# SymbioticLab/Oobleck

Measured on AMD Instinct MI355X. Metric: tokens/sec (whole node) GPT-2 1F1B, higher is better.
Workload: dtype bf16; 1 GPU; gpt2.yaml GPT-2-small 1F1B, global microbatch 128x1024 tokens, bf16; model=gpt2, global_batch=128, seq_len=1024, parallelism=pp1dp1

## Files before the change

### include/oobleck_stage.h

```cpp
#ifndef OOBLECK_STAGE_H
#define OOBLECK_STAGE_H

#include <stdint.h>

#ifdef __cplusplus
extern "C" {
#endif

enum {
  OB_KIND_EMBED = 0,
  OB_KIND_BLOCK = 1,
  OB_KIND_FINAL = 2
};

typedef struct ob_layer* ob_layer_t;

typedef struct {
  int32_t kind;
  int32_t n_embd;
  int32_t n_head;
  int32_t n_positions;
  int32_t vocab_size;
  int32_t max_batch;
  int32_t seq_len;
  int32_t n_slots;
  int32_t dtype;
} ob_layer_desc;

int64_t ob_layer_param_count(const ob_layer_desc* desc);

int ob_layer_create(const ob_layer_desc* desc, ob_layer_t* out);

enum {
  OB_DROP_EMBD = 0,
  OB_DROP_ATTN = 1,
  OB_DROP_RESID_ATTN = 2,
  OB_DROP_RESID_MLP = 3
};

typedef struct {
  float embd_pdrop;
  float resid_pdrop;
  float attn_pdrop;
  int32_t layer_id;
  uint64_t seed;
} ob_dropout_desc;

int ob_layer_create_ex(const ob_layer_desc* desc, const ob_dropout_desc* drop,
                       ob_layer_t* out);

int ob_layer_uses_flash(ob_layer_t l);
int ob_flash_eligible(const ob_layer_desc* desc, float attn_pdrop);

int ob_layer_plan_query(const ob_layer_desc* desc,
                        const ob_dropout_desc* drop, int modes, int64_t* out,
                        int cap);

int ob_layer_set_training(ob_layer_t l, int on);

int ob_layer_set_dropout_tick(ob_layer_t l, uint64_t tick);

int ob_layer_bind(ob_layer_t l, void* params, void* grads);

int ob_layer_set_batch(ob_layer_t l, int32_t batch);

int ob_layer_forward(ob_layer_t l, int32_t slot, const void* in, void* out,
                     const int64_t* labels, void* stream);

int ob_layer_backward(ob_layer_t l, int32_t slot, const void* dout, void* din,
                      void* stream);

int ob_layer_destroy(ob_layer_t l);

int ob_layer_refresh_weights(ob_layer_t l, void* stream);

int ob_adamw_step(void* p, const void* g, void* m, void* v, int64_t n,
                  int32_t step, float lr, float beta1, float beta2, float eps,
                  float weight_decay, void* stream);


int64_t ob_sqnorm_ws_count(const int64_t* counts, int32_t n);

int ob_sqnorm_multi_f32(const void* const* ptrs, const int64_t* counts,
                        const int32_t* out_index, int32_t n, void* ws,
                        void* out, void* stream);

int ob_clip_finish(const void* sq, int32_t n, float max_norm, void* stats,
                   void* stream);

int ob_adamw_step_scaled(void* p, const void* g, void* m, void* v, int64_t n,
                         int32_t step, float lr, float beta1, float beta2,
                         float eps, float weight_decay, const void* clip_stats,
                         void* stream);


int ob_gemm_f32(int transA, int transB, int64_t M, int64_t N, int64_t K,
                float alpha, const void* A, int64_t lda,
                int64_t strideA1, int64_t strideA2,
                const void* B, int64_t ldb,
                int64_t strideB1, int64_t strideB2,
                float beta, void* C, int64_t ldc,
                int64_t strideC1, int64_t strideC2,
                int64_t n1, int64_t n2,
                const void* bias, const void* residual, int atomic, int splitk,
                void* stream);

int ob_layernorm_fwd_f32(const void* x, const void* w, const void* b, void* y,
                         void* mean, void* rstd, int64_t rows, int64_t H,
                         float eps, void* stream);
int ob_layernorm_bwd_f32(const void* x, const void* w, const void* mean,
                         const void* rstd, const void* dy, void* dx,
                         void* dw, void* db, int64_t rows, int64_t H,
                         int dx_accum, void* stream);

int ob_softmax_causal_fwd_f32(void* scores, int64_t batch, int64_t S,
                              float scale, void* stream);
int ob_softmax_causal_bwd_f32(const void* P, void* dP, int64_t batch,
                              int64_t S, void* stream);

int ob_gelu_fwd_f32(const void* u, void* g, int64_t n, void* stream);
int ob_gelu_bwd_f32(const void* u, const void* dg, void* du, int64_t n,
                    void* stream);

int ob_colsum_f32(const void* X, void* db, int64_t M, int64_t N, void* stream);

int ob_dropout_mask(uint64_t seed, int32_t layer_id, int32_t site,
                    uint64_t tick, float p, int64_t n, void* keep_u8,
                    void* stream);
int ob_dropout_scale_f32(uint64_t seed, int32_t layer_id, int32_t site,
                         uint64_t tick, float p, const void* x, void* y,
                         int64_t n, void* stream);
int ob_dropout_scale_bf16(uint64_t seed, int32_t layer_id, int32_t site,
                          uint64_t tick, float p, const void* x, void* y,
                          int64_t n, void* stream);
int ob_dropout_add_f32(uint64_t seed, int32_t layer_id, int32_t site,
                       uint64_t tick, float p, const void* t, const void* res,
                       void* y, int64_t n, void* stream);
int ob_dropout_add_bf16(uint64_t seed, int32_t layer_id, int32_t site,
                        uint64_t tick, float p, const void* t,
                        const void* res, void* y, int64_t n, void* stream);
int ob_dropout_scale_colsum_f32(uint64_t seed, int32_t layer_id, int32_t site,
                                uint64_t tick, float p, const void* dy,
                                void* dm, void* db, int64_t M, int64_t N,
                                void* stream);
int ob_dropout_scale_colsum_bf16(uint64_t seed, int32_t layer_id, int32_t site,
                                 uint64_t tick, float p, const void* dy,
                                 void* dm, void* db, int64_t M, int64_t N,
                                 void* stream);

int ob_gemm_bf16(int transA, int transB, int64_t M, int64_t N, int64_t K,
                 float alpha, const void* A, int64_t lda,
                 int64_t strideA1, int64_t strideA2,
                 const void* B, int64_t ldb,
                 int64_t strideB1, int64_t strideB2,
                 float beta, void* C, int64_t ldc,
                 int64_t strideC1, int64_t strideC2,
                 int64_t n1, int64_t n2,
                 const void* bias, const void* residual, int out_kind,
                 int splitk, void* stream);
int ob_gemm_bf16_route(int transA, int transB, int64_t M, int64_t N, int64_t K,
                       int64_t n1, int64_t n2, int out_kind, int splitk,
                       float beta, int aligned16, int env_mask,
                       const char* force, int32_t* out);

int ob_layer_lt_shapes(const ob_layer_desc* desc, int64_t* out, int cap);
int ob_gemm_lt_tune(const int64_t* shape);
int ob_gemm_lt_choice(const int64_t* shape, double* out, char* top1_name,
                      char* chosen_name, int name_cap);
int ob_gemm_lt_candidates(const int64_t* shape, int32_t* index, int32_t* pos,
                          double* us, int cap);
int64_t ob_gemm_lt_table_size(void);
int64_t ob_gemm_lt_untuned_uses(void);
int ob_gemm_lt_plan_index(const int64_t* shape, void* stream);

int ob_flash_fwd_nt_bf16(const void* qkv, void* O, void* lse, int64_t B,
                         int64_t Sq, int64_t H, int64_t nh, float scale,
                         void* stream);
int ob_flash_bwd_nt_bf16(const void* qkv, const void* dO, const void* lse,
                         const void* D, void* dqkv, void* dbias_qkv,
                         int64_t B, int64_t Sq, int64_t H, int64_t nh,
                         float scale, void* stream);
int ob_flash_bwd_nt_d_bf16(const void* qkv, const void* O, const void* dO,
                           const void* lse, void* D_ws, void* dqkv,
                           void* dbias_qkv, int64_t B, int64_t Sq, int64_t H,
                           int64_t nh, float scale, void* stream);
int ob_flash_fwd_nt_drop_bf16(const void* qkv, void* O, void* lse, int64_t B,
                              int64_t Sq, int64_t H, int64_t nh, float scale,
                              uint64_t seed, int32_t layer_id, uint64_t tick,
                              float p, void* stream);
int ob_flash_bwd_nt_d_drop_bf16(const void* qkv, const void* O, const void* dO,
                                const void* lse, void* D_ws, void* dqkv,
                                void* dbias_qkv, int64_t B, int64_t Sq,
                                int64_t H, int64_t nh, float scale,
                                uint64_t seed, int32_t layer_id, uint64_t tick,
                                float p, void* stream);
int ob_flash_fold_rows(int64_t kind, int64_t Sq, int64_t block, int64_t unit,
                       int64_t* row0, int64_t* first_tile, int64_t* n_tiles);
int64_t ob_flash_fold_grid(int64_t kind, int64_t Sq, int64_t Z);
int ob_flash_fold_id(int64_t kind, int64_t Sq, int64_t Z, int64_t id,
                     int64_t* z, int64_t* block);

int ob_set_deterministic(int on);
int ob_deterministic(void);

enum {
  OB_DET_WS_COLSUM = 0,
  OB_DET_WS_GELU = 1,
  OB_DET_WS_LN = 2,
  OB_DET_WS_DROP_CS = 3,
  OB_DET_WS_CE = 4
};
int64_t ob_det_ws_count(int which, int64_t M, int64_t N);
int ob_colsum_det_bf16(const void* X, void* db, int64_t M, int64_t N,
                       void* ws, void* stream);
int ob_gelu_bwd_colsum_det_bf16(const void* u, const void* dg, void* du,
                                void* db, int64_t M, int64_t N, void* ws,
                                void* stream);
int ob_layernorm_bwd_res_det_bf16(const void* x, const void* w,
                                  const void* mean, const void* rstd,
                                  const void* dy, const void* res, void* dx,
                                  void* dw, void* db, void* sum_res,
                                  void* sum_dx, int64_t rows, int64_t H,
                                  void* ws, void* stream);
int ob_dropout_scale_colsum_det_bf16(uint64_t seed, int32_t layer_id,
                                     int32_t site, uint64_t tick, float p,
                                     const void* dy, void* dm, void* db,
                                     int64_t M, int64_t N, void* ws,
                                     void* stream);
int ob_ce_fwd_det_bf16(const void* logits, const void* labels, void* lse,
                       void* loss, int64_t B, int64_t Sq, int64_t V,
                       int64_t ld, void* ws, void* stream);
int ob_embed_bwd_det_bf16(const void* ids, const void* dout, void* dwte,
                          void* dwpe, int64_t B, int64_t Sq, int64_t H,
                          void* stream);
int ob_embed_bwd_drop_det_bf16(uint64_t seed, int32_t layer_id, int32_t site,
                               uint64_t tick, float p, const void* ids,
                               const void* dout, void* dwte, void* dwpe,
                               int64_t B, int64_t Sq, int64_t H, void* stream);
int ob_colpart_finish_f32(const void* part, int64_t nblk, int64_t N,
                          int64_t ld, void* dst, void* stream);

int ob_f32_to_bf16(const void* x, void* y, int64_t n, void* stream);
int ob_f32_to_bf16_t(const void* x, void* y, int64_t rows, int64_t cols,
                     void* stream);
int ob_bf16_to_f32(const void* x, void* y, int64_t n, void* stream);

void ob_profile_enable(int on);
void ob_profile_reset(void);
int ob_profile_read(int fam, double* total_ms, long long* count);

const char* ob_last_error(void);

const char* ob_build_arch(void);

#ifdef __cplusplus
}
#endif
#endif
```

### oobleck_amd/_ext.py

```python
from __future__ import annotations

import ctypes
import pathlib

_LIB = None
SO_PATH = pathlib.Path(__file__).resolve().parent / "libob_stage.so"


class ObLayerDesc(ctypes.Structure):
    _fields_ = [
        ("kind", ctypes.c_int32),
        ("n_embd", ctypes.c_int32),
        ("n_head", ctypes.c_int32),
        ("n_positions", ctypes.c_int32),
        ("vocab_size", ctypes.c_int32),
        ("max_batch", ctypes.c_int32),
        ("seq_len", ctypes.c_int32),
        ("n_slots", ctypes.c_int32),
        ("dtype", ctypes.c_int32),
    ]


class ObDropoutDesc(ctypes.Structure):
    _fields_ = [
        ("embd_pdrop", ctypes.c_float),
        ("resid_pdrop", ctypes.c_float),
        ("attn_pdrop", ctypes.c_float),
        ("layer_id", ctypes.c_int32),
        ("seed", ctypes.c_uint64),
    ]


DROP_EMBD, DROP_ATTN, DROP_RESID_ATTN, DROP_RESID_MLP = 0, 1, 2, 3


def _configure(lib: ctypes.CDLL) -> ctypes.CDLL:
    i64, i32, f32, vp = ctypes.c_int64, ctypes.c_int32, ctypes.c_float, ctypes.c_void_p
    lib.ob_last_error.restype = ctypes.c_char_p
    lib.ob_build_arch.restype = ctypes.c_char_p
    lib.ob_layer_param_count.restype = i64
    lib.ob_layer_param_count.argtypes = [ctypes.POINTER(ObLayerDesc)]
    lib.ob_layer_create.argtypes = [ctypes.POINTER(ObLayerDesc),
                                    ctypes.POINTER(vp)]
    u64 = ctypes.c_uint64
    lib.ob_layer_create_ex.argtypes = [ctypes.POINTER(ObLayerDesc),
                                       ctypes.POINTER(ObDropoutDesc),
                                       ctypes.POINTER(vp)]
    lib.ob_layer_set_training.argtypes = [vp, i32]
    lib.ob_layer_uses_flash.argtypes = [vp]
    lib.ob_flash_eligible.argtypes = [ctypes.POINTER(ObLayerDesc), f32]
    lib.ob_layer_plan_query.argtypes = [ctypes.POINTER(ObLayerDesc),
                                        ctypes.POINTER(ObDropoutDesc), i32,
                                        ctypes.POINTER(i64), i32]
    lib.ob_layer_set_dropout_tick.argtypes = [vp, u64]
    key = [u64, i32, i32, u64, f32]
    lib.ob_dropout_mask.argtypes = key + [i64, vp, vp]
    lib.ob_dropout_scale_f32.argtypes = key + [vp, vp, i64, vp]
    lib.ob_dropout_scale_bf16.argtypes = key + [vp, vp, i64, vp]
    lib.ob_dropout_add_f32.argtypes = key + [vp, vp, vp, i64, vp]
    lib.ob_dropout_add_bf16.argtypes = key + [vp, vp, vp, i64, vp]
    lib.ob_dropout_scale_colsum_f32.argtypes = key + [vp, vp, vp, i64, i64, vp]
    lib.ob_dropout_scale_colsum_bf16.argtypes = key + [vp, vp, vp, i64, i64,
                                                       vp]
    lib.ob_layer_bind.argtypes = [vp, vp, vp]
    lib.ob_layer_set_batch.argtypes = [vp, i32]
    lib.ob_layer_forward.argtypes = [vp, i32, vp, vp, vp, vp]
    lib.ob_layer_backward.argtypes = [vp, i32, vp, vp, vp]
    lib.ob_layer_destroy.argtypes = [vp]
    lib.ob_layer_refresh_weights.argtypes = [vp, vp]
    lib.ob_adamw_step.argtypes = [vp, vp, vp, vp, i64, i32, f32, f32, f32,
                                  f32, f32, vp]
    lib.ob_sqnorm_ws_count.restype = i64
    lib.ob_sqnorm_ws_count.argtypes = [ctypes.POINTER(i64), i32]
    lib.ob_sqnorm_multi_f32.argtypes = [ctypes.POINTER(vp),
                                        ctypes.POINTER(i64),
                                        ctypes.POINTER(i32), i32, vp, vp, vp]
    lib.ob_clip_finish.argtypes = [vp, i32, f32, vp, vp]
    lib.ob_adamw_step_scaled.argtypes = [vp, vp, vp, vp, i64, i32, f32, f32,
                                         f32, f32, f32, vp, vp]
    lib.ob_gemm_f32.argtypes = [i32, i32, i64, i64, i64, f32, vp, i64, i64,
                                i64, vp, i64, i64, i64, f32, vp, i64, i64,
                                i64, i64, i64, vp, vp, i32, i32, vp]
    lib.ob_layernorm_fwd_f32.argtypes = [vp, vp, vp, vp, vp, vp, i64, i64,
                                         f32, vp]
    lib.ob_layernorm_bwd_f32.argtypes = [vp, vp, vp, vp, vp, vp, vp, vp, i64,
                                         i64, i32, vp]
    lib.ob_softmax_causal_fwd_f32.argtypes = [vp, i64, i64, f32, vp]
    lib.ob_softmax_causal_bwd_f32.argtypes = [vp, vp, i64, i64, vp]
    lib.ob_gelu_fwd_f32.argtypes = [vp, vp, i64, vp]
    lib.ob_gelu_bwd_f32.argtypes = [vp, vp, vp, i64, vp]
    lib.ob_colsum_f32.argtypes = [vp, vp, i64, i64, vp]
    lib.ob_gemm_bf16.argtypes = [i32, i32, i64, i64, i64, f32, vp, i64, i64,
                                 i64, vp, i64, i64, i64, f32, vp, i64, i64,
                                 i64, i64, i64, vp, vp, i32, i32, vp]
    lib.ob_f32_to_bf16.argtypes = [vp, vp, i64, vp]
    lib.ob_f32_to_bf16_t.argtypes = [vp, vp, i64, i64, vp]
    lib.ob_f32_to_bf16_t_ld.argtypes = [vp, vp, i64, i64, i64, vp]
    lib.ob_bf16_to_f32.argtypes = [vp, vp, i64, vp]
    lib.ob_gelu_fwd_bf16.argtypes = [vp, vp, i64, vp]
    lib.ob_gelu_bwd_bf16.argtypes = [vp, vp, vp, i64, vp]
    lib.ob_ce_fwd_bf16.argtypes = [vp, vp, vp, vp, i64, i64, i64, i64, vp]
    lib.ob_ce_bwd_bf16.argtypes = [vp, vp, vp, vp, i64, i64, i64, i64, vp]
    lib.ob_embed_fwd_bf16.argtypes = [vp, vp, vp, vp, i64, i64, i64, vp]
    lib.ob_embed_bwd_bf16.argtypes = [vp, vp, vp, vp, i64, i64, i64, vp]
    lib.ob_softmax_causal_fwd_bf16.argtypes = [vp, i64, i64, f32, vp]
    lib.ob_softmax_causal_bwd_bf16.argtypes = [vp, vp, i64, i64, vp]
    lib.ob_transpose_bf16.argtypes = [vp, vp, i64, i64, vp]
    lib.ob_gemm_lt_bias.argtypes = [i32, i32, i64, i64, i64, f32, vp, i64,
                                    vp, i64, f32, vp, i64, i32, vp, vp]
    lib.ob_gemm_lt_f32.argtypes = [i32, i32, i64, i64, i64, f32, vp, i64,
                                   vp, i64, f32, vp, i64, vp]
    lib.ob_flash_fwd_bf16.argtypes = [vp, vp, vp, vp, i64, i64, i64, i64,
                                      f32, vp]
    lib.ob_transpose_bf16_b.argtypes = [vp, vp, i64, i64, i64, i64, i64,
                                        i64, i64, vp]
    lib.ob_layernorm_fwd_bf16.argtypes = [vp, vp, vp, vp, vp, vp, i64, i64,
                                          f32, vp]
    lib.ob_layernorm_bwd_bf16.argtypes = [vp, vp, vp, vp, vp, vp, vp, vp,
                                          i64, i64, i32, vp]
    lib.ob_colsum_bf16.argtypes = [vp, vp, i64, i64, vp]
    lib.ob_layernorm_fwd_copy_bf16.argtypes = [vp, vp, vp, vp, vp, vp, vp,
                                               i64, i64, f32, vp]
    lib.ob_layernorm_bwd_res_bf16.argtypes = [vp, vp, vp, vp, vp, vp, vp, vp,
                                              vp, vp, vp, i64, i64, vp]
    lib.ob_gelu_bwd_colsum_bf16.argtypes = [vp, vp, vp, vp, i64, i64, vp]
    lib.ob_gemm_lt.argtypes = [i32, i32, i64, i64, i64, f32, vp, i64, vp,
                               i64, f32, vp, i64, i32, vp]
    lib.ob_gemm_bf16_nt_8ph.argtypes = [vp, vp, vp, vp, vp, i64, i64, i64,
                                        i64, i64, i64, i64, i64, i64, i64,
                                        i64, i64, i64, i64, f32, f32, i32,
                                        i32, vp, i64]
    lib.ob_gemm_bf16_route.argtypes = [i32, i32, i64, i64, i64, i64, i64, i32,
                                       i32, f32, i32, i32, ctypes.c_char_p,
                                       ctypes.POINTER(ctypes.c_int32)]
    lib.ob_gemm_lt_bias_res.argtypes = [i32, i32, i64, i64, i64, f32, vp, i64,
                                        vp, i64, vp, i64, i32, vp, vp, vp]
    shape = ctypes.POINTER(i64)
    lib.ob_layer_lt_shapes.argtypes = [ctypes.POINTER(ObLayerDesc), shape, i32]
    lib.ob_gemm_lt_tune.argtypes = [shape]
    lib.ob_gemm_lt_choice.argtypes = [shape, ctypes.POINTER(ctypes.c_double),
                                      ctypes.c_char_p, ctypes.c_char_p, i32]
    lib.ob_gemm_lt_candidates.argtypes = [shape, ctypes.POINTER(i32),
                                          ctypes.POINTER(i32),
                                          ctypes.POINTER(ctypes.c_double), i32]
    lib.ob_gemm_lt_table_size.argtypes = []
    lib.ob_gemm_lt_table_size.restype = i64
    lib.ob_gemm_lt_untuned_uses.argtypes = []
    lib.ob_gemm_lt_untuned_uses.restype = i64
    lib.ob_gemm_lt_plan_index.argtypes = [shape, vp]
    lib.ob_profile_enable.argtypes = [i32]
    lib.ob_profile_enable.restype = None
    lib.ob_profile_reset.argtypes = []
    lib.ob_profile_reset.restype = None
    lib.ob_profile_read.argtypes = [i32, ctypes.POINTER(ctypes.c_double),
                                    ctypes.POINTER(ctypes.c_longlong)]
    lib.ob_flash_dsum_bf16.argtypes = [vp, vp, vp, i64, i64, i64, i64, vp]
    lib.ob_flash_bwd_bf16.argtypes = [vp, vp, vp, vp, vp, vp, vp, vp, i64,
                                      i64, i64, i64, f32, vp]
    lib.ob_flash_fwd_nt_bf16.argtypes = [vp, vp, vp, i64, i64, i64, i64,
                                         f32, vp]
    lib.ob_flash_bwd_nt_bf16.argtypes = [vp, vp, vp, vp, vp, vp, i64, i64,
                                         i64, i64, f32, vp]
    lib.ob_flash_bwd_nt_d_bf16.argtypes = [vp, vp, vp, vp, vp, vp, vp, i64,
                                           i64, i64, i64, f32, vp]
    lib.ob_flash_fwd_nt_drop_bf16.argtypes = [vp, vp, vp, i64, i64, i64, i64,
                                              f32, u64, i32, u64, f32, vp]
    lib.ob_flash_bwd_nt_d_drop_bf16.argtypes = [vp, vp, vp, vp, vp, vp, vp,
                                                i64, i64, i64, i64, f32, u64,
                                                i32, u64, f32, vp]
    lib.ob_set_deterministic.argtypes = [i32]
    lib.ob_deterministic.argtypes = []
    lib.ob_det_ws_count.argtypes = [i32, i64, i64]
    lib.ob_det_ws_count.restype = i64
    lib.ob_colsum_det_bf16.argtypes = [vp, vp, i64, i64, vp, vp]
    lib.ob_gelu_bwd_colsum_det_bf16.argtypes = [vp, vp, vp, vp, i64, i64, vp,
                                                vp]
    lib.ob_layernorm_bwd_res_det_bf16.argtypes = [vp, vp, vp, vp, vp, vp, vp,
                                                  vp, vp, vp, vp, i64, i64,
                                                  vp, vp]
    lib.ob_dropout_scale_colsum_det_bf16.argtypes = key + [vp, vp, vp, i64,
                                                           i64, vp, vp]
    lib.ob_ce_fwd_det_bf16.argtypes = [vp, vp, vp, vp, i64, i64, i64, i64,
                                       vp, vp]
    lib.ob_embed_bwd_det_bf16.argtypes = [vp, vp, vp, vp, i64, i64, i64, vp]
    lib.ob_embed_bwd_drop_det_bf16.argtypes = key + [vp, vp, vp, vp, i64,
                                                     i64, i64, vp]
    lib.ob_colpart_finish_f32.argtypes = [vp, i64, i64, i64, vp, vp]
    p64 = ctypes.POINTER(ctypes.c_int64)
    lib.ob_flash_fold_rows.argtypes = [i64, i64, i64, i64, p64, p64, p64]
    lib.ob_flash_fold_grid.argtypes = [i64, i64, i64]
    lib.ob_flash_fold_grid.restype = ctypes.c_int64
    lib.ob_flash_fold_id.argtypes = [i64, i64, i64, i64, p64, p64]
    return lib


def get_ext(build_if_missing: bool = True) -> ctypes.CDLL:
    global _LIB
    if _LIB is not None:
        return _LIB
    if not SO_PATH.exists():
        if build_if_missing:
            from .build import build
            try:
                build()
            except Exception as e:
                raise RuntimeError(
                    f"oobleck_amd: HIP extension missing and build failed: {e}. "
                    "The hot path has no fallback — run __graft_entry__.build().") from e
        else:
            raise RuntimeError(
                "oobleck_amd: HIP extension libob_stage.so is missing. "
                "The hot path has no fallback — run __graft_entry__.build().")
    _LIB = _configure(ctypes.CDLL(str(SO_PATH)))
    return _LIB


LT_SHAPE_FIELDS = 13
LT_SHAPE_NAMES = ("tA", "tB", "M", "N", "K", "lda", "ldb", "ldc", "c_f32",
                  "beta1", "bias", "cin", "ab_f32")


def lt_shape(tA, tB, M, N, K, lda, ldb, ldc, c_f32=0, beta1=0, bias=0, cin=0,
             ab_f32=0):
    return (ctypes.c_int64 * LT_SHAPE_FIELDS)(tA, tB, M, N, K, lda, ldb, ldc,
                                              c_f32, beta1, bias, cin, ab_f32)


def layer_lt_shapes(desc: ObLayerDesc) -> list[tuple]:
    lib = get_ext()
    n = lib.ob_layer_lt_shapes(ctypes.byref(desc), None, 0)
    if n < 0:
        raise RuntimeError("ob_layer_lt_shapes failed")
    buf = (ctypes.c_int64 * (LT_SHAPE_FIELDS * max(n, 1)))()
    lib.ob_layer_lt_shapes(ctypes.byref(desc), buf, n)
    return [tuple(buf[i * LT_SHAPE_FIELDS:(i + 1) * LT_SHAPE_FIELDS])
            for i in range(n)]


def lt_choice(shape) -> dict | None:
    out = (ctypes.c_double * 10)()
    top1 = ctypes.create_string_buffer(512)
    chosen = ctypes.create_string_buffer(512)
    check(get_ext().ob_gemm_lt_choice(lt_shape(*shape), out, top1, chosen, 512),
          "gemm_lt_choice")
    if not out[0]:
        return None
    return {"index": int(out[1]), "tuned": bool(out[2]),
            "top1_index": int(out[3]), "us_top1": out[4], "us_chosen": out[5],
            "tried": int(out[6]), "dropped": int(out[7]), "wall_ms": out[8],
            "spread_top1": out[9],
            "top1_kernel": top1.value.decode(),
            "chosen_kernel": chosen.value.decode()}


def lt_candidates(shape, cap: int = 128) -> list[dict]:
    idx, pos = (ctypes.c_int32 * cap)(), (ctypes.c_int32 * cap)()
    us = (ctypes.c_double * cap)()
    n = get_ext().ob_gemm_lt_candidates(lt_shape(*shape), idx, pos, us, cap)
    return [{"index": idx[i], "pos": pos[i], "us": us[i]}
            for i in range(max(0, min(n, cap)))]


PLAN_STASH = ("x", "mean1", "rstd1", "ln1", "qkv", "p", "attnm", "hmid",
              "mean2", "rstd2", "ln2", "u", "g", "logits", "lse")
PLAN_SHADOWS = ("qkv", "qkv_t", "ap", "ap_t", "fc", "fc_t", "mp", "mp_t",
                "lm", "lm_t")
PLAN_WS = ("dp", "dln", "datt", "dqkv", "dy4", "flash_bwd", "flash_vt",
           "dw_a", "dw_b", "pd_fwd", "pd_bwd", "dm_attn", "dm_mlp",
           "det_main", "det_side", "det_fwd")
LAYER_PLAN_NAMES = (
    ("flash", "side", "v_pad", "slot_stride", "ids_count", "shadow_count")
    + tuple(f"st_off_{n}" for n in PLAN_STASH)
    + tuple(f"st_len_{n}" for n in PLAN_STASH)
    + tuple(f"sh_off_{n}" for n in PLAN_SHADOWS)
    + tuple(f"ws_{n}" for n in PLAN_WS)
    + ("pk_qt", "pk_kt", "pk_dot", "pk_d"))
PLAN_DET, PLAN_BF16_FLASH, PLAN_FLASH_TR, PLAN_FLASH_DROP, PLAN_FLASH_HD128 = (
    1, 2, 4, 8, 16)


def layer_plan(desc: ObLayerDesc, drop: ObDropoutDesc | None = None,
               modes: int = -1) -> dict:
    n = len(LAYER_PLAN_NAMES)
    buf = (ctypes.c_int64 * n)()
    got = get_ext().ob_layer_plan_query(
        ctypes.byref(desc), ctypes.byref(drop) if drop else None, modes, buf,
        n)
    if got != n:
        raise RuntimeError(f"ob_layer_plan_query returned {got}, not {n}")
    return dict(zip(LAYER_PLAN_NAMES, buf))


DET_WS_COLSUM, DET_WS_GELU, DET_WS_LN, DET_WS_DROP_CS, DET_WS_CE = range(5)


def set_deterministic(on: bool) -> None:
    check(get_ext().ob_set_deterministic(1 if on else 0), "set_deterministic")


def deterministic() -> bool:
    return bool(get_ext().ob_deterministic())


def check(rc: int, what: str = "") -> None:
    if rc != 0:
        err = get_ext().ob_last_error().decode()
        raise RuntimeError(f"oobleck_amd extension error in {what}: {err}")
```

### oobleck_amd/build.py

```python
from __future__ import annotations

import pathlib
import subprocess

PKG_DIR = pathlib.Path(__file__).resolve().parent
SO_PATH = PKG_DIR / "libob_stage.so"
SOURCES = [PKG_DIR / "csrc" / "ob_kernels.hip",
           PKG_DIR / "csrc" / "ob_kernels_bf16.hip",
           PKG_DIR / "csrc" / "ob_gemm_bf16.hip",
           PKG_DIR / "csrc" / "ob_flash_bf16.hip",
           PKG_DIR / "csrc" / "ob_flash_hd128_bf16.hip",
           PKG_DIR / "csrc" / "ob_blaslt.hip",
           PKG_DIR / "csrc" / "ob_optim.hip",
           PKG_DIR / "csrc" / "ob_dropout.hip",
           PKG_DIR / "csrc" / "ob_layer.hip"]
HEADERS = [PKG_DIR.parent / "include" / "oobleck_stage.h",
           PKG_DIR / "csrc" / "ob_internal.h",
           PKG_DIR / "csrc" / "ob_layer_plan.h",
           PKG_DIR / "csrc" / "ob_flash_fold.h",
           PKG_DIR / "csrc" / "ob_flash_common.h",
           PKG_DIR / "csrc" / "ob_bf16.h",
           PKG_DIR / "csrc" / "ob_gemm_route.h",
           PKG_DIR / "csrc" / "ob_philox.h"]


def needs_rebuild() -> bool:
    if not SO_PATH.exists():
        return True
    so_mtime = SO_PATH.stat().st_mtime
    return any(p.stat().st_mtime > so_mtime for p in SOURCES + HEADERS)


def build(force: bool = False) -> pathlib.Path:
    if force or needs_rebuild():
        cmd = ["hipcc", "--offload-arch=gfx950", "-O3", "-std=c++17", "-fPIC",
               "-shared"] + [str(s) for s in SOURCES] + \
              ["-L/opt/rocm/lib", "-lhipblaslt", "-o", str(SO_PATH)]
        subprocess.run(cmd, check=True, capture_output=True, text=True)
    return SO_PATH


if __name__ == "__main__":
    print(build(force=True))
```

### oobleck_amd/csrc/ob_blaslt.hip

```cpp
#include "ob_internal.h"

#include <hipblaslt/hipblaslt-ext.hpp>
#include <hipblaslt/hipblaslt.h>

#include <algorithm>
#include <atomic>
#include <chrono>
#include <cstdlib>
#include <cstring>
#include <map>
#include <mutex>
#include <set>
#include <string>
#include <tuple>
#include <vector>

namespace {

constexpr size_t kLtWs = 64u << 20;

struct Key {
  ob_lt_shape s;
  auto tie() const {
    return std::tie(s.tA, s.tB, s.M, s.N, s.K, s.lda, s.ldb, s.ldc, s.c_f32,
                    s.beta1, s.bias, s.cin, s.ab_f32);
  }
  bool operator<(const Key& o) const { return tie() < o.tie(); }
};

struct LtProblem {
  hipblasLtMatmulDesc_t desc = nullptr;
  hipblasLtMatrixLayout_t la = nullptr, lb = nullptr, lc = nullptr;
};

struct LtPlan {
  LtProblem p;
  hipblasLtMatmulAlgo_t algo{};
  int index = -1;
  bool ok = false;
  bool untuned = false;
};

struct LtCtx {
  hipblasLtHandle_t h = nullptr;
  void* ws = nullptr;
  std::map<Key, LtPlan> plans;
};
std::map<void*, LtCtx> g_lt_by_stream;

struct LtChoice {
  int index = -1;
  int top1_index = -1;
  bool tuned = false;
  double us_top1 = 0, us_chosen = 0;
  int tried = 0, dropped = 0;
  double wall_ms = 0;
  double spread_top1 = 0;
  std::string top1_name, chosen_name;
  struct Timed {
    int index, pos;
    double us;
  };
  std::vector<Timed> timed;
};
std::mutex g_tab_mu;
std::map<Key, LtChoice> g_tab;
std::atomic<int64_t> g_untuned_uses{0};

bool lt_tune_on() {
  static const bool on = ob_env_flag("OB_LT_TUNE", true);
  return on && !ob_deterministic();
}

LtCtx* lt_ctx(void* stream) {
  auto it = g_lt_by_stream.find(stream);
  if (it != g_lt_by_stream.end()) return &it->second;
  LtCtx ctx;
  if (hipblasLtCreate(&ctx.h) != HIPBLAS_STATUS_SUCCESS) return nullptr;
  if (hipMalloc(&ctx.ws, kLtWs) != hipSuccess) return nullptr;
  return &g_lt_by_stream.emplace(stream, ctx).first->second;
}

void lt_problem_create(const ob_lt_shape& k, const void* bias, LtProblem* p) {
  const hipblasOperation_t opA = k.tB ? HIPBLAS_OP_T : HIPBLAS_OP_N;
  const hipblasOperation_t opB = k.tA ? HIPBLAS_OP_T : HIPBLAS_OP_N;
  const int64_t a_rows = k.tB ? k.K : k.N, a_cols = k.tB ? k.N : k.K;
  const int64_t b_rows = k.tA ? k.M : k.K, b_cols = k.tA ? k.K : k.M;
  hipblasLtMatmulDescCreate(&p->desc, HIPBLAS_COMPUTE_32F, HIP_R_32F);
  hipblasLtMatmulDescSetAttribute(p->desc, HIPBLASLT_MATMUL_DESC_TRANSA, &opA,
                                  sizeof(opA));
  hipblasLtMatmulDescSetAttribute(p->desc, HIPBLASLT_MATMUL_DESC_TRANSB, &opB,
                                  sizeof(opB));
  if (k.bias) {
    const hipblasLtEpilogue_t ep = HIPBLASLT_EPILOGUE_BIAS;
    hipblasLtMatmulDescSetAttribute(p->desc, HIPBLASLT_MATMUL_DESC_EPILOGUE,
                                    &ep, sizeof(ep));
    const int32_t bt = HIP_R_32F;
    hipblasLtMatmulDescSetAttribute(
        p->desc, HIPBLASLT_MATMUL_DESC_BIAS_DATA_TYPE, &bt, sizeof(bt));
    hipblasLtMatmulDescSetAttribute(
        p->desc, HIPBLASLT_MATMUL_DESC_BIAS_POINTER, &bias, sizeof(bias));
  }
  const hipDataType abt = k.ab_f32 ? HIP_R_32F : HIP_R_16BF;
  hipblasLtMatrixLayoutCreate(&p->la, abt, a_rows, a_cols, k.ldb);
  hipblasLtMatrixLayoutCreate(&p->lb, abt, b_rows, b_cols, k.lda);
  hipblasLtMatrixLayoutCreate(&p->lc, k.c_f32 ? HIP_R_32F : HIP_R_16BF, k.N,
                              k.M, k.ldc);
}

void lt_problem_destroy(LtProblem* p) {
  if (p->la) hipblasLtMatrixLayoutDestroy(p->la);
  if (p->lb) hipblasLtMatrixLayoutDestroy(p->lb);
  if (p->lc) hipblasLtMatrixLayoutDestroy(p->lc);
  if (p->desc) hipblasLtMatmulDescDestroy(p->desc);
  *p = LtProblem();
}

int lt_heuristic(hipblasLtHandle_t h, const LtProblem& p, int n,
                 hipblasLtMatmulHeuristicResult_t* res) {
  hipblasLtMatmulPreference_t pref;
  hipblasLtMatmulPreferenceCreate(&pref);
  const uint64_t ws = kLtWs;
  hipblasLtMatmulPreferenceSetAttribute(
      pref, HIPBLASLT_MATMUL_PREF_MAX_WORKSPACE_BYTES, &ws, sizeof(ws));
  int nres = 0;
  const hipblasStatus_t st = hipblasLtMatmulAlgoGetHeuristic(
      h, p.desc, p.la, p.lb, p.lc, p.lc, pref, n, res, &nres);
  hipblasLtMatmulPreferenceDestroy(pref);
  return st == HIPBLAS_STATUS_SUCCESS ? nres : 0;
}

bool lt_algo_from_index(hipblasLtHandle_t h, const LtProblem& p,
                        const ob_lt_shape& k, int index,
                        hipblasLtMatmulAlgo_t* algo) {
  std::vector<int> idx{index};
  std::vector<hipblasLtMatmulHeuristicResult_t> r;
  if (hipblaslt_ext::getAlgosFromIndex(h, idx, r) != HIPBLAS_STATUS_SUCCESS ||
      r.empty())
    return false;
  const float alpha = 1.f, beta = k.beta1 ? 1.f : 0.f;
  size_t need = 0;
  if (hipblaslt_ext::matmulIsAlgoSupported(h, p.desc, &alpha, p.la, p.lb,
                                           &beta, p.lc, p.lc, r[0].algo,
                                           need) != HIPBLAS_STATUS_SUCCESS ||
      need > kLtWs)
    return false;
  *algo = r[0].algo;
  return true;
}

LtPlan lt_plan_build(LtCtx* ctx, const Key& key, const void* bias) {
  LtPlan p;
  lt_problem_create(key.s, bias, &p.p);
  int index = -1;
  {
    std::lock_guard<std::mutex> lk(g_tab_mu);
    auto it = g_tab.find(key);
    if (it == g_tab.end())
      p.untuned = lt_tune_on();
    else if (it->second.tuned && lt_tune_on())
      index = it->second.index;
  }
  if (index >= 0 && lt_algo_from_index(ctx->h, p.p, key.s, index, &p.algo)) {
    p.index = index;
    p.ok = true;
    return p;
  }
  hipblasLtMatmulHeuristicResult_t res[1];
  if (lt_heuristic(ctx->h, p.p, 1, res) > 0 &&
      res[0].state == HIPBLAS_STATUS_SUCCESS) {
    p.algo = res[0].algo;
    p.index = hipblaslt_ext::getIndexFromAlgo(p.algo);
    p.ok = true;
  }
  return p;
}


__global__ void k_lt_fill(void* p, int64_t n, int f32, uint32_t seed) {
  for (int64_t i = blockIdx.x * (int64_t)blockDim.x + threadIdx.x; i < n;
       i += (int64_t)gridDim.x * blockDim.x) {
    uint32_t h = (uint32_t)i * 2654435761u + (uint32_t)(i >> 32) + seed;
    h ^= h >> 16, h *= 0x7feb352du, h ^= h >> 15, h *= 0x846ca68bu;
    h ^= h >> 16;
    const float v = (float)(h >> 16) * (1.f / 32768.f) - 1.f;
    if (f32) ((float*)p)[i] = v;
    else ((__bf16*)p)[i] = (__bf16)v;
  }
}

__global__ void k_lt_diff(const void* x, const void* ref, int64_t n, int f32,
                          double* acc) {
  double d2 = 0, r2 = 0;
  for (int64_t i = blockIdx.x * (int64_t)blockDim.x + threadIdx.x; i < n;
       i += (int64_t)gridDim.x * blockDim.x) {
    const float a = f32 ? ((const float*)x)[i] : (float)((const __bf16*)x)[i];
    const float b =
        f32 ? ((const float*)ref)[i] : (float)((const __bf16*)ref)[i];
    d2 += (double)(a - b) * (a - b);
    r2 += (double)b * b;
  }
  __shared__ double sd[256], sr[256];
  sd[threadIdx.x] = d2, sr[threadIdx.x] = r2;
  __syncthreads();
  for (int s = 128; s > 0; s >>= 1) {
    if ((int)threadIdx.x < s) {
      sd[threadIdx.x] += sd[threadIdx.x + s];
      sr[threadIdx.x] += sr[threadIdx.x + s];
    }
    __syncthreads();
  }
  if (threadIdx.x == 0) {
    atomicAdd(&acc[0], sd[0]);
    atomicAdd(&acc[1], sr[0]);
  }
}

double median_of(std::vector<float> v) {
  std::sort(v.begin(), v.end());
  return v[v.size() / 2];
}

struct TuneScratch {
  hipStream_t stream = nullptr;
  hipblasLtHandle_t h = nullptr;
  void *ws = nullptr, *A = nullptr, *B = nullptr, *C = nullptr, *Cref = nullptr,
       *Cin = nullptr, *bias = nullptr;
  double* acc = nullptr;
  hipEvent_t e0 = nullptr, e1 = nullptr;
  LtProblem p;
  ~TuneScratch() {
    lt_problem_destroy(&p);
    for (void* q : {ws, A, B, C, Cref, Cin, bias, (void*)acc})
      if (q) (void)hipFree(q);
    if (e0) (void)hipEventDestroy(e0);
    if (e1) (void)hipEventDestroy(e1);
    if (h) hipblasLtDestroy(h);
    if (stream) (void)hipStreamDestroy(stream);
  }
};

struct Cand {
  hipblasLtMatmulAlgo_t algo;
  int pos = 0;
  int reps = 1;
  float warm_us = 0.f;
  std::vector<float> us;
};

bool lt_tune_run(const ob_lt_shape& k, LtChoice* out) {
  const int n_env = ob_env_int("OB_LT_TUNE_N", 8);
  const int n_max = n_env < 1 ? 1 : n_env > 128 ? 128 : n_env;
  constexpr int kRounds = 5;
  TuneScratch t;
#define LT_TRY(x) \
  if ((x) != hipSuccess) return false
  LT_TRY(hipStreamCreateWithFlags(&t.stream, hipStreamNonBlocking));
  if (hipblasLtCreate(&t.h) != HIPBLAS_STATUS_SUCCESS) return false;
  LT_TRY(hipEventCreate(&t.e0));
  LT_TRY(hipEventCreate(&t.e1));
  const size_t es_ab = k.ab_f32 ? 4 : 2, es_c = k.c_f32 ? 4 : 2;
  const int64_t nA = (k.tA ? k.K : k.M) * k.lda;
  const int64_t nB = (k.tB ? k.N : k.K) * k.ldb;
  const int64_t nC = k.M * k.ldc;
  LT_TRY(hipMalloc(&t.ws, kLtWs));
  LT_TRY(hipMalloc(&t.A, nA * es_ab));
  LT_TRY(hipMalloc(&t.B, nB * es_ab));
  LT_TRY(hipMalloc(&t.C, nC * es_c));
  LT_TRY(hipMalloc(&t.Cref, nC * es_c));
  LT_TRY(hipMalloc((void**)&t.acc, 2 * sizeof(double)));
  if (k.cin) LT_TRY(hipMalloc(&t.Cin, nC * es_c));
  if (k.bias) LT_TRY(hipMalloc(&t.bias, k.N * sizeof(float)));
  auto fill = [&](void* p, int64_t n, int f32, uint32_t seed) {
    const int64_t blocks = std::min<int64_t>((n + 255) / 256, 4096);
    k_lt_fill<<<(unsigned)blocks, 256, 0, t.stream>>>(p, n, f32, seed);
  };
  fill(t.A, nA, k.ab_f32, 1u);
  fill(t.B, nB, k.ab_f32, 2u);
  if (t.Cin) fill(t.Cin, nC, k.c_f32, 3u);
  if (t.bias) fill(t.bias, k.N, 1, 4u);
  LT_TRY(hipGetLastError());
  lt_problem_create(k, t.bias, &t.p);

  std::vector<hipblasLtMatmulHeuristicResult_t> res(n_max);
  res.resize(std::max(0, lt_heuristic(t.h, t.p, n_max, res.data())));
  if (res.empty() || res[0].state != HIPBLAS_STATUS_SUCCESS) return false;
  out->top1_index = hipblaslt_ext::getIndexFromAlgo(res[0].algo);
  out->top1_name = hipblaslt_ext::getKernelNameFromAlgo(t.h, res[0].algo);

  const float alpha = 1.f, beta = k.beta1 ? 1.f : 0.f;
  if (ob_env_flag("OB_LT_TUNE_ALL", false)) {
    std::vector<hipblasLtMatmulHeuristicResult_t> every;
    const hipDataType abt = k.ab_f32 ? HIP_R_32F : HIP_R_16BF;
    const hipDataType ct = k.c_f32 ? HIP_R_32F : HIP_R_16BF;
    if (hipblaslt_ext::getAllAlgos(
            t.h, hipblaslt_ext::GemmType::HIPBLASLT_GEMM,
            k.tB ? HIPBLAS_OP_T : HIPBLAS_OP_N,
            k.tA ? HIPBLAS_OP_T : HIPBLAS_OP_N, abt, abt, ct, ct,
            HIPBLAS_COMPUTE_32F, every) == HIPBLAS_STATUS_SUCCESS) {
      std::set<int> seen;
      for (auto& r : res) seen.insert(hipblaslt_ext::getIndexFromAlgo(r.algo));
      for (auto& r : every) {
        size_t need = 0;
        if (!seen.insert(hipblaslt_ext::getIndexFromAlgo(r.algo)).second)
          continue;
        if (hipblaslt_ext::matmulIsAlgoSupported(
                t.h, t.p.desc, &alpha, t.p.la, t.p.lb, &beta, t.p.lc, t.p.lc,
                r.algo, need) != HIPBLAS_STATUS_SUCCESS ||
            need > kLtWs)
          continue;
        r.state = HIPBLAS_STATUS_SUCCESS;
        res.push_back(r);
      }
    }
  }
  const int nres = (int)res.size();
  auto run = [&](hipblasLtMatmulAlgo_t& algo, void* dst) {
    return hipblasLtMatmul(t.h, t.p.desc, &alpha, t.B, t.p.la, t.A, t.p.lb,
                           &beta, t.Cin ? t.Cin : dst, t.p.lc, dst, t.p.lc,
                           &algo, t.ws, kLtWs, t.stream);
  };
  const double bound = k.c_f32 ? 1e-3 : 1.0 / 256;
  std::vector<Cand> cands;
  for (int i = 0; i < nres; i++) {
    if (res[i].state != HIPBLAS_STATUS_SUCCESS) {
      out->dropped++;
      continue;
    }
    void* dst = i == 0 ? t.Cref : t.C;
    LT_TRY(hipMemsetAsync(dst, 0, nC * es_c, t.stream));
    const hipblasStatus_t st = run(res[i].algo, dst);
    if (i == 0 && st != HIPBLAS_STATUS_SUCCESS) return false;
    if (st != HIPBLAS_STATUS_SUCCESS) {
      LT_TRY(hipStreamSynchronize(t.stream));
      out->dropped++;
      continue;
    }
    if (i > 0) {
      LT_TRY(hipMemsetAsync(t.acc, 0, 2 * sizeof(double), t.stream));
      const int64_t blocks = std::min<int64_t>((nC + 255) / 256, 4096);
      k_lt_diff<<<(unsigned)blocks, 256, 0, t.stream>>>(t.C, t.Cref, nC,
                                                        k.c_f32, t.acc);
      double acc[2] = {0, 0};
      LT_TRY(hipMemcpyAsync(acc, t.acc, sizeof(acc), hipMemcpyDeviceToHost,
                            t.stream));
      LT_TRY(hipStreamSynchronize(t.stream));
      if (!(acc[0] <= bound * bound * acc[1])) {
        out->dropped++;
        continue;
      }
    } else {
      LT_TRY(hipStreamSynchronize(t.stream));
    }
    Cand c;
    c.algo = res[i].algo;
    c.pos = i;
    cands.push_back(c);
  }
  out->tried = nres;
  enum { V_OK = 0, V_DROP = 1, V_HIP = 2 };
  auto visit = [&](Cand& c, int reps, float* us) {
    if (hipEventRecord(t.e0, t.stream) != hipSuccess) return (int)V_HIP;
    bool lib_ok = true;
    for (int r = 0; r < reps && lib_ok; r++)
      lib_ok = run(c.algo, t.C) == HIPBLAS_STATUS_SUCCESS;
    float ms = 0.f;
    if (hipEventRecord(t.e1, t.stream) != hipSuccess ||
        hipEventSynchronize(t.e1) != hipSuccess ||
        hipEventElapsedTime(&ms, t.e0, t.e1) != hipSuccess)
      return (int)V_HIP;
    if (!lib_ok) return (int)V_DROP;
    *us = ms * 1000.f / reps;
    return (int)V_OK;
  };
  auto drop = [&](size_t i) {
    if (i == 0) return false;
    cands.erase(cands.begin() + i);
    out->dropped++;
    return true;
  };
  auto reps_for = [](float us) {
    return std::max(1, std::min(4096, (int)(1250.f / std::max(us, 0.25f)) + 1));
  };
  LT_TRY(hipMemsetAsync(t.C, 0, nC * es_c, t.stream));
  for (size_t i = 0; i < cands.size();) {
    Cand& c = cands[i];
    float us = 0.f;
    int v = visit(c, 1, &us);
    if (v == V_OK) v = visit(c, 8, &us);
    if (v == V_HIP || (v == V_DROP && !drop(i))) return false;
    if (v == V_DROP) continue;
    c.warm_us = us;
    c.reps = reps_for(us);
    i++;
  }
  if ((int)cands.size() > n_max) {
    std::stable_sort(cands.begin() + 1, cands.end(),
                     [](const Cand& a, const Cand& b) {
                       return a.warm_us < b.warm_us;
                     });
    cands.resize(n_max);
  }
  for (int r = 0; r < kRounds; r++)
    for (size_t i = 0; i < cands.size();) {
      Cand& c = cands[i];
      float us = 0.f;
      int v = V_OK;
      for (int attempt = 0; attempt < 4; attempt++) {
        v = visit(c, c.reps, &us);
        if (v != V_OK || us * c.reps >= 1000.f || c.reps >= 4096) break;
        c.reps = std::max(c.reps + 1, reps_for(us));
      }
      if (v == V_HIP || (v == V_DROP && !drop(i))) return false;
      if (v == V_DROP) continue;
      c.us.push_back(us);
      i++;
    }
  LT_TRY(hipStreamSynchronize(t.stream));
#undef LT_TRY
  const double med0 = median_of(cands[0].us);
  const double spread0 =
      *std::max_element(cands[0].us.begin(), cands[0].us.end()) -
      *std::min_element(cands[0].us.begin(), cands[0].us.end());
  size_t best = 0;
  double best_med = med0;
  out->timed.push_back(
      {hipblaslt_ext::getIndexFromAlgo(cands[0].algo), 0, med0});
  for (size_t i = 1; i < cands.size(); i++) {
    const double m = median_of(cands[i].us);
    out->timed.push_back(
        {hipblaslt_ext::getIndexFromAlgo(cands[i].algo), cands[i].pos, m});
    if (m < best_med) best_med = m, best = i;
  }
  out->spread_top1 = spread0;
  const double min0 =
      *std::min_element(cands[0].us.begin(), cands[0].us.end());
  if (!(best_med < med0 - spread0) ||
      !(*std::max_element(cands[best].us.begin(), cands[best].us.end()) <
        min0))
    best = 0, best_med = med0;
  out->us_top1 = med0;
  out->us_chosen = best_med;
  out->index = hipblaslt_ext::getIndexFromAlgo(cands[best].algo);
  out->chosen_name = hipblaslt_ext::getKernelNameFromAlgo(t.h, cands[best].algo);
  out->tuned = true;
  return true;
}

Key key_from_i64(const int64_t* v) {
  Key key;
  ob_lt_shape& s = key.s;
  s.tA = v[0] != 0, s.tB = v[1] != 0, s.M = v[2], s.N = v[3], s.K = v[4];
  s.lda = v[5], s.ldb = v[6], s.ldc = v[7], s.c_f32 = v[8] != 0;
  s.beta1 = v[9] != 0, s.bias = v[10] != 0, s.cin = v[11] != 0;
  s.ab_f32 = v[12] != 0;
  return key;
}

}

int ob_lt_tune_shape(const ob_lt_shape& s) {
  if (!lt_tune_on()) return 0;
  if (s.M <= 0 || s.N <= 0 || s.K <= 0 || s.ldc < s.N ||
      s.lda < (s.tA ? s.M : s.K) || s.ldb < (s.tB ? s.K : s.N))
    return ob_fail("lt_tune: bad shape");
  const Key key{s};
  {
    std::lock_guard<std::mutex> lk(g_tab_mu);
    if (g_tab.count(key)) return 0;
  }
  OB_HIP(hipDeviceSynchronize());
  const auto t0 = std::chrono::steady_clock::now();
  LtChoice c;
  if (!lt_tune_run(s, &c)) {
    c.tuned = false;
    c.index = c.top1_index;
    (void)hipGetLastError();
  }
  (void)hipDeviceSynchronize();
  c.wall_ms = std::chrono::duration<double, std::milli>(
                  std::chrono::steady_clock::now() - t0)
                  .count();
  {
    std::lock_guard<std::mutex> lk(g_tab_mu);
    g_tab.emplace(key, c);
  }
  for (auto& sc : g_lt_by_stream) {
    auto it = sc.second.plans.find(key);
    if (it == sc.second.plans.end()) continue;
    lt_problem_destroy(&it->second.p);
    sc.second.plans.erase(it);
  }
  return 0;
}

static int lt_matmul(int tA, int tB, int64_t M, int64_t N, int64_t K,
                     float alpha, const void* A, int64_t lda, const void* B,
                     int64_t ldb, float beta, void* C, int64_t ldc,
                     int c_f32, const void* bias, int ab_f32, void* stream,
                     const void* Cin = nullptr) {
  if (!Cin) Cin = C;
  LtCtx* ctx = lt_ctx(stream);
  if (!ctx) return ob_fail("hipblasLt per-stream context init failed");
  const Key key{ob_lt_shape_of(tA, tB, M, N, K, lda, ldb, ldc, c_f32, beta,
                               bias != nullptr, Cin != C, ab_f32)};
  auto it = ctx->plans.find(key);
  if (it == ctx->plans.end())
    it = ctx->plans.emplace(key, lt_plan_build(ctx, key, bias)).first;
  const LtPlan& p = it->second;
  if (!p.ok) return -1;
  if (p.untuned) g_untuned_uses.fetch_add(1, std::memory_order_relaxed);
  if (bias)
    hipblasLtMatmulDescSetAttribute(
        p.p.desc, HIPBLASLT_MATMUL_DESC_BIAS_POINTER, &bias, sizeof(bias));
  const hipblasStatus_t st = hipblasLtMatmul(
      ctx->h, p.p.desc, &alpha, B, p.p.la, A, p.p.lb, &beta, Cin, p.p.lc, C,
      p.p.lc, &p.algo, ctx->ws, kLtWs, reinterpret_cast<hipStream_t>(stream));
  if (st != HIPBLAS_STATUS_SUCCESS)
    return ob_fail("hipblasLtMatmul failed (%d)", (int)st);
  return 0;
}

extern "C" int ob_gemm_lt(int tA, int tB, int64_t M, int64_t N, int64_t K,
                          float alpha, const void* A, int64_t lda,
                          const void* B, int64_t ldb, float beta, void* C,
                          int64_t ldc, int c_f32, void* stream) {
  return lt_matmul(tA, tB, M, N, K, alpha, A, lda, B, ldb, beta, C, ldc,
                   c_f32, nullptr, 0, stream);
}

extern "C" int ob_gemm_lt_bias(int tA, int tB, int64_t M, int64_t N,
                               int64_t K, float alpha, const void* A,
                               int64_t lda, const void* B, int64_t ldb,
                               float beta, void* C, int64_t ldc, int c_f32,
                               const void* bias, void* stream) {
  return lt_matmul(tA, tB, M, N, K, alpha, A, lda, B, ldb, beta, C, ldc,
                   c_f32, bias, 0, stream);
}

extern "C" int ob_gemm_lt_bias_res(int tA, int tB, int64_t M, int64_t N,
                                   int64_t K, float alpha, const void* A,
                                   int64_t lda, const void* B, int64_t ldb,
                                   void* C, int64_t ldc, int c_f32,
                                   const void* bias, const void* residual,
                                   void* stream) {
  return lt_matmul(tA, tB, M, N, K, alpha, A, lda, B, ldb, 1.f, C, ldc,
                   c_f32, bias, 0, stream, residual);
}

extern "C" int ob_gemm_lt_f32(int tA, int tB, int64_t M, int64_t N,
                              int64_t K, float alpha, const void* A,
                              int64_t lda, const void* B, int64_t ldb,
                              float beta, void* C, int64_t ldc,
                              void* stream) {
  return lt_matmul(tA, tB, M, N, K, alpha, A, lda, B, ldb, beta, C, ldc, 1,
                   nullptr, 1, stream);
}


extern "C" int ob_gemm_lt_tune(const int64_t* shape) {
  if (!shape) return ob_fail("gemm_lt_tune: null shape");
  return ob_lt_tune_shape(key_from_i64(shape).s);
}

extern "C" int ob_gemm_lt_choice(const int64_t* shape, double* out,
                                 char* top1_name, char* chosen_name,
                                 int name_cap) {
  if (!shape || !out) return ob_fail("gemm_lt_choice: null argument");
  const Key key = key_from_i64(shape);
  std::lock_guard<std::mutex> lk(g_tab_mu);
  auto it = g_tab.find(key);
  for (int i = 0; i < 10; i++) out[i] = 0;
  if (top1_name && name_cap > 0) top1_name[0] = 0;
  if (chosen_name && name_cap > 0) chosen_name[0] = 0;
  if (it == g_tab.end()) return 0;
  const LtChoice& c = it->second;
  out[0] = 1, out[1] = c.index, out[2] = c.tuned, out[3] = c.top1_index;
  out[4] = c.us_top1, out[5] = c.us_chosen, out[6] = c.tried;
  out[7] = c.dropped, out[8] = c.wall_ms, out[9] = c.spread_top1;
  if (top1_name && name_cap > 0)
    snprintf(top1_name, name_cap, "%s", c.top1_name.c_str());
  if (chosen_name && name_cap > 0)
    snprintf(chosen_name, name_cap, "%s", c.chosen_name.c_str());
  return 0;
}

extern "C" int ob_gemm_lt_candidates(const int64_t* shape, int32_t* index,
                                     int32_t* pos, double* us, int cap) {
  if (!shape || (cap > 0 && (!index || !pos || !us))) return -1;
  std::lock_guard<std::mutex> lk(g_tab_mu);
  auto it = g_tab.find(key_from_i64(shape));
  if (it == g_tab.end()) return 0;
  auto v = it->second.timed;
  std::stable_sort(v.begin(), v.end(),
                   [](const LtChoice::Timed& a, const LtChoice::Timed& b) {
                     return a.us < b.us;
                   });
  for (int i = 0; i < (int)v.size() && i < cap; i++)
    index[i] = v[i].index, pos[i] = v[i].pos, us[i] = v[i].us;
  return (int)v.size();
}

extern "C" int64_t ob_gemm_lt_table_size(void) {
  std::lock_guard<std::mutex> lk(g_tab_mu);
  return (int64_t)g_tab.size();
}

extern "C" int64_t ob_gemm_lt_untuned_uses(void) {
  return g_untuned_uses.load(std::memory_order_relaxed);
}

extern "C" int ob_gemm_lt_plan_index(const int64_t* shape, void* stream) {
  if (!shape) return -1;
  auto sc = g_lt_by_stream.find(stream);
  if (sc == g_lt_by_stream.end()) return -1;
  auto it = sc->second.plans.find(key_from_i64(shape));
  return it == sc->second.plans.end() || !it->second.ok ? -1
                                                        : it->second.index;
}
```

### oobleck_amd/csrc/ob_internal.h

```cpp
#pragma once
#include <hip/hip_runtime.h>

#include <cstdarg>
#include <cstdint>
#include <cstdio>
#include <cstdlib>

#include "../../include/oobleck_stage.h"

int ob_fail(const char* fmt, ...);

#define OB_HIP(x)                                                     \
  do {                                                                \
    hipError_t e_ = (x);                                              \
    if (e_ != hipSuccess)                                             \
      return ob_fail("%s:%d: %s", __FILE__, __LINE__,                 \
                     hipGetErrorString(e_));                          \
  } while (0)

#define OB_LAUNCH_CHECK()                                             \
  do {                                                                \
    hipError_t e_ = hipGetLastError();                                \
    if (e_ != hipSuccess)                                             \
      return ob_fail("%s:%d: launch: %s", __FILE__, __LINE__,         \
                     hipGetErrorString(e_));                          \
  } while (0)

inline bool ob_env_flag(const char* name, bool dflt) {
  const char* e = getenv(name);
  return (e && e[0] == (dflt ? '0' : '1')) ? !dflt : dflt;
}
inline int ob_env_int(const char* name, int dflt) {
  const char* e = getenv(name);
  return e ? atoi(e) : dflt;
}

enum {
  OB_PF_FC_FWD = 0,
  OB_PF_GEMM_FWD = 1,
  OB_PF_GEMM_DX = 2,
  OB_PF_GEMM_DW = 3,
  OB_PF_FLASH_FWD = 4,
  OB_PF_FLASH_BWD = 5,
  OB_PF_ATTN_MAT = 6,
  OB_PF_LN = 7,
  OB_PF_CE = 8,
  OB_PF_ELEM = 9,
  OB_PF_ADAMW = 10,
  OB_PF_NFAM = 11
};
bool ob_prof_on();
int ob_prof_beg(int fam, hipStream_t s);
void ob_prof_end(int fam, int slot, hipStream_t s);

#define OB_PROF(fid, strm, call)                                        \
  ({                                                                    \
    int _r;                                                             \
    if (ob_prof_on()) {                                                 \
      hipStream_t _ps = reinterpret_cast<hipStream_t>(strm);            \
      const int _fi = (fid);                                            \
      const int _slot = ob_prof_beg(_fi, _ps);                          \
      _r = (call);                                                      \
      ob_prof_end(_fi, _slot, _ps);                                     \
    } else {                                                            \
      _r = (call);                                                      \
    }                                                                   \
    _r;                                                                 \
  })

__device__ __forceinline__ void ob_adamw_update(
    float* __restrict__ p, float* __restrict__ m, float* __restrict__ v,
    int64_t i, float gi, float wd_factor, float step_size, float inv_sqrt_bc2,
    float beta1, float beta2, float eps) {
  float mi = beta1 * m[i] + (1.f - beta1) * gi;
  float vi = beta2 * v[i] + (1.f - beta2) * gi * gi;
  m[i] = mi;
  v[i] = vi;
  const float denom = sqrtf(vi) * inv_sqrt_bc2 + eps;
  p[i] = p[i] * wd_factor - step_size * mi / denom;
}

int ob_embed_fwd_f32(const int64_t* ids, const float* wte, const float* wpe,
                     float* out, int64_t B, int64_t S, int64_t H, void* stream);
int ob_embed_bwd_f32(const int64_t* ids, const float* dout, float* dwte,
                     float* dwpe, int64_t B, int64_t S, int64_t H, void* stream);
int ob_ce_fwd_f32(const float* logits, const int64_t* labels, float* lse,
                  float* loss, int64_t B, int64_t S, int64_t V, void* stream);
int ob_ce_bwd_f32(float* logits_to_dlogits, const int64_t* labels,
                  const float* lse, const float* dloss_or_null, int64_t B,
                  int64_t S, int64_t V, void* stream);

struct ob_drop_key;
int ob_drop_scale(const ob_drop_key& key, int bf16, const void* x, void* y,
                  int64_t n, void* stream);
int ob_drop_add(const ob_drop_key& key, int bf16, const void* t,
                const void* res, void* y, int64_t n, void* stream);
int ob_drop_scale_colsum(const ob_drop_key& key, int bf16, const void* dy,
                         void* dm, void* db, int64_t M, int64_t N,
                         void* stream, float* ws = nullptr);
int ob_embed_fwd_drop(const ob_drop_key& key, int bf16, const int64_t* ids,
                      const float* wte, const float* wpe, void* out, int64_t B,
                      int64_t Sq, int64_t H, void* stream);
int ob_embed_bwd_drop(const ob_drop_key& key, int bf16, const int64_t* ids,
                      const void* dout, float* dwte, float* dwpe, int64_t B,
                      int64_t Sq, int64_t H, void* stream);
int64_t ob_drop_cs_ws_count(int64_t M, int64_t N);
int ob_embed_bwd_det(const ob_drop_key* key, const int64_t* ids,
                     const void* dout, float* dwte, float* dwpe, int64_t B,
                     int64_t Sq, int64_t H, void* stream);

extern "C" {
int ob_f32_to_bf16_t_ld(const void* x, void* y, int64_t rows, int64_t cols,
                        int64_t out_ld, void* stream);
int ob_layernorm_fwd_bf16(const void* x, const void* w, const void* b,
                          void* y, void* mean, void* rstd, int64_t rows,
                          int64_t H, float eps, void* stream);
int ob_layernorm_bwd_bf16(const void* x, const void* w, const void* mean,
                          const void* rstd, const void* dy, void* dx,
                          void* dw, void* db, int64_t rows, int64_t H,
                          int dx_accum, void* stream);
int ob_layernorm_fwd_copy_bf16(const void* x, const void* w, const void* b,
                               void* y, void* xcopy, void* mean, void* rstd,
                               int64_t rows, int64_t H, float eps,
                               void* stream);
int ob_layernorm_bwd_res_bf16(const void* x, const void* w, const void* mean,
                              const void* rstd, const void* dy,
                              const void* res, void* dx, void* dw, void* db,
                              void* sum_res, void* sum_dx, int64_t rows,
                              int64_t H, void* stream);
int ob_gelu_bwd_colsum_bf16(const void* u, const void* dg, void* du,
                            void* db, int64_t M, int64_t N, void* stream);
int ob_softmax_causal_fwd_bf16(void* scores, int64_t batch, int64_t Sq,
                               float scale, void* stream);
int ob_softmax_causal_bwd_bf16(const void* P, void* dP, int64_t batch,
                               int64_t Sq, void* stream);
int ob_gelu_fwd_bf16(const void* u, void* g, int64_t n, void* stream);
int ob_gelu_bwd_bf16(const void* u, const void* dg, void* du, int64_t n,
                     void* stream);
int ob_colsum_bf16(const void* X, void* db, int64_t M, int64_t N,
                   void* stream);
int ob_embed_fwd_bf16(const void* ids, const void* wte, const void* wpe,
                      void* out, int64_t B, int64_t Sq, int64_t H,
                      void* stream);
int ob_embed_bwd_bf16(const void* ids, const void* dout, void* dwte,
                      void* dwpe, int64_t B, int64_t Sq, int64_t H,
                      void* stream);
int ob_ce_fwd_bf16(const void* logits, const void* labels, void* lse,
                   void* loss, int64_t B, int64_t Sq, int64_t V, int64_t ld,
                   void* stream);
int ob_ce_bwd_bf16(void* logits, const void* labels, const void* lse,
                   const void* dloss, int64_t B, int64_t Sq, int64_t V,
                   int64_t ld, void* stream);
int ob_transpose_bf16(const void* in, void* out, int64_t R, int64_t C,
                      void* stream);
int ob_flash_fwd_bf16(const void* qkv, const void* VT, void* O, void* lse,
                      int64_t B, int64_t Sq, int64_t H, int64_t nh,
                      float scale, void* stream);
int ob_transpose_bf16_b(const void* in, void* out, int64_t R, int64_t C,
                        int64_t sIn1, int64_t sIn2, int64_t ldin, int64_t n1,
                        int64_t n2, void* stream);
int ob_flash_dsum_bf16(const void* O, const void* dO, void* D, int64_t B,
                       int64_t Sq, int64_t H, int64_t nh, void* stream);
int ob_flash_bwd_bf16(const void* qkv, const void* QT, const void* KT,
                      const void* dOT, const void* dO, const void* lse,
                      const void* D, void* dqkv, int64_t B, int64_t Sq,
                      int64_t H, int64_t nh, float scale, void* stream);
int ob_flash_fwd_nt_bf16(const void* qkv, void* O, void* lse, int64_t B,
                         int64_t Sq, int64_t H, int64_t nh, float scale,
                         void* stream);
int ob_flash_bwd_nt_bf16(const void* qkv, const void* dO, const void* lse,
                         const void* D, void* dqkv, void* dbias_qkv,
                         int64_t B, int64_t Sq, int64_t H, int64_t nh,
                         float scale, void* stream);
int ob_flash_bwd_nt_d_bf16(const void* qkv, const void* O, const void* dO,
                           const void* lse, void* D_ws, void* dqkv,
                           void* dbias_qkv, int64_t B, int64_t Sq, int64_t H,
                           int64_t nh, float scale, void* stream);
}
int ob_layernorm_bwd_ws(const void* x, const void* w, const void* mean,
                        const void* rstd, const void* dy, void* dx, void* dw,
                        void* db, int64_t rows, int64_t H, int dx_accum,
                        float* ws, void* stream);
int ob_layernorm_bwd_res_ws(const void* x, const void* w, const void* mean,
                            const void* rstd, const void* dy, const void* res,
                            void* dx, void* dw, void* db, void* sum_res,
                            void* sum_dx, int64_t rows, int64_t H, float* ws,
                            void* stream);
int ob_colsum_ws(const void* X, void* db, int64_t M, int64_t N, float* ws,
                 void* stream);
int ob_gelu_bwd_colsum_ws(const void* u, const void* dg, void* du, void* db,
                          int64_t M, int64_t N, float* ws, void* stream);
int ob_ce_fwd_ws(const void* logits, const void* labels, void* lse,
                 void* loss, int64_t B, int64_t Sq, int64_t V, int64_t ld,
                 float* ws, void* stream);
extern "C" int ob_gemm_lt(int tA, int tB, int64_t M, int64_t N, int64_t K,
                          float alpha, const void* A, int64_t lda,
                          const void* B, int64_t ldb, float beta, void* C,
                          int64_t ldc, int c_f32, void* stream);
extern "C" int ob_gemm_lt_bias(int tA, int tB, int64_t M, int64_t N,
                               int64_t K, float alpha, const void* A,
                               int64_t lda, const void* B, int64_t ldb,
                               float beta, void* C, int64_t ldc, int c_f32,
                               const void* bias, void* stream);
extern "C" int ob_gemm_lt_bias_res(int tA, int tB, int64_t M, int64_t N,
                                   int64_t K, float alpha, const void* A,
                                   int64_t lda, const void* B, int64_t ldb,
                                   void* C, int64_t ldc, int c_f32,
                                   const void* bias, const void* residual,
                                   void* stream);
extern "C" int ob_gemm_lt_f32(int tA, int tB, int64_t M, int64_t N,
                              int64_t K, float alpha, const void* A,
                              int64_t lda, const void* B, int64_t ldb,
                              float beta, void* C, int64_t ldc,
                              void* stream);
struct ob_lt_shape {
  int tA = 0, tB = 0;
  int64_t M = 0, N = 0, K = 0, lda = 0, ldb = 0, ldc = 0;
  int c_f32 = 0;
  int beta1 = 0;
  int bias = 0;
  int cin = 0;
  int ab_f32 = 0;
};
#define OB_LT_SHAPE_FIELDS 13
inline ob_lt_shape ob_lt_shape_of(int tA, int tB, int64_t M, int64_t N,
                                  int64_t K, int64_t lda, int64_t ldb,
                                  int64_t ldc, int c_f32, float beta,
                                  bool bias, bool cin, int ab_f32) {
  ob_lt_shape s;
  s.tA = tA != 0, s.tB = tB != 0, s.M = M, s.N = N, s.K = K;
  s.lda = lda, s.ldb = ldb, s.ldc = ldc, s.c_f32 = c_f32 != 0;
  s.beta1 = beta != 0.f, s.bias = bias, s.cin = cin, s.ab_f32 = ab_f32 != 0;
  return s;
}
inline ob_lt_shape ob_lt_linear(int64_t M, int64_t K, int64_t N, bool bias,
                                bool res) {
  return ob_lt_shape_of(0, 1, M, N, K, K, K, N, 0, res ? 1.f : 0.f, bias, res,
                        0);
}
inline ob_lt_shape ob_lt_dw(int64_t actw, int64_t dyw, int64_t BS,
                            int64_t lda) {
  return ob_lt_shape_of(1, 0, actw, dyw, BS, lda, dyw, dyw, 1, 1.f, false,
                        false, 0);
}
int ob_lt_tune_shape(const ob_lt_shape& s);

struct ob_bf16_gemm {
  const void* A = nullptr;
  const void* B = nullptr;
  void* C = nullptr;
  const void* bias = nullptr;
  const void* residual = nullptr;
  int64_t M = 0, N = 0, K = 0;
  int64_t lda = 0, ldb = 0, ldc = 0;
  int64_t sA1 = 0, sA2 = 0, sB1 = 0, sB2 = 0, sC1 = 0, sC2 = 0;
  int64_t n1 = 1, n2 = 1;
  float alpha = 1.f, beta = 0.f;
  int transA = 0, transB = 1;
  int out_kind = 0;
  int splitk = 1;
  int64_t Mr = 0;
  void* stream = nullptr;
};
int ob_gemm_bf16_run(const ob_bf16_gemm& g);
int ob_gemm_bf16_nt_dispatch(const ob_bf16_gemm& g);
int ob_gemm_bf16_nt256_dispatch(const ob_bf16_gemm& g, int BN);
int ob_gemm_bf16_nt_8ph_dispatch(const ob_bf16_gemm& g);
```

### oobleck_amd/csrc/ob_layer.hip

```cpp
#include "ob_gemm_route.h"
#include "ob_internal.h"
#include "ob_layer_plan.h"
#include "ob_philox.h"

#include <atomic>
#include <cmath>
#include <cstring>
#include <initializer_list>
#include <memory>
#include <vector>

static inline hipStream_t S(void* s) { return reinterpret_cast<hipStream_t>(s); }


static struct {
  float* buf[WS_N];
  int64_t size[WS_N];
} g_ws;
template <class T>
static T* ws(int i) { return reinterpret_cast<T*>(g_ws.buf[i]); }

struct SideSync {
  hipStream_t stream = nullptr;
  hipEvent_t ring[128] = {};
  int ri = 0;
  bool ready = false;
};
static SideSync g_side;

static hipEvent_t side_evt() {
  hipEvent_t e = g_side.ring[g_side.ri & 127];
  g_side.ri++;
  return e;
}

static int side_init() {
  if (g_side.ready) return 0;
  OB_HIP(hipStreamCreateWithFlags(&g_side.stream, hipStreamNonBlocking));
  for (int i = 0; i < 128; i++)
    OB_HIP(hipEventCreateWithFlags(&g_side.ring[i], hipEventDisableTiming));
  g_side.ready = true;
  return 0;
}

#define OB_SIDE_FENCE(from, to)                      \
  do {                                               \
    hipEvent_t ev_ = side_evt();                     \
    OB_HIP(hipEventRecord(ev_, (from)));             \
    OB_HIP(hipStreamWaitEvent((to), ev_, 0));        \
  } while (0)


struct ProfFam {
  static constexpr int RING = 64;
  hipEvent_t beg[RING] = {}, end[RING] = {};
  bool pending[RING] = {};
  int head = 0;
  double total_ms = 0.0;
  long long count = 0;
};
static struct {
  bool on = false;
  ProfFam fam[OB_PF_NFAM];
} g_prof;

static void prof_drain_slot(ProfFam& f, int i) {
  if (!f.pending[i]) return;
  hipEventSynchronize(f.end[i]);
  float ms = 0.f;
  if (hipEventElapsedTime(&ms, f.beg[i], f.end[i]) == hipSuccess)
    f.total_ms += ms;
  f.pending[i] = false;
}

bool ob_prof_on() { return g_prof.on; }

int ob_prof_beg(int fam, hipStream_t s) {
  ProfFam& f = g_prof.fam[fam];
  const int i = f.head;
  if (!f.beg[i]) {
    hipEventCreate(&f.beg[i]);
    hipEventCreate(&f.end[i]);
  }
  prof_drain_slot(f, i);
  hipEventRecord(f.beg[i], s);
  return i;
}

void ob_prof_end(int fam, int slot, hipStream_t s) {
  ProfFam& f = g_prof.fam[fam];
  hipEventRecord(f.end[slot], s);
  f.pending[slot] = true;
  f.count++;
  f.head = (slot + 1) % ProfFam::RING;
}

extern "C" void ob_profile_enable(int on) { g_prof.on = on != 0; }

extern "C" void ob_profile_reset(void) {
  for (auto& f : g_prof.fam) {
    for (int i = 0; i < ProfFam::RING; i++)
      if (f.pending[i]) {
        hipEventSynchronize(f.end[i]);
        f.pending[i] = false;
      }
    f.total_ms = 0.0;
    f.count = 0;
    f.head = 0;
  }
}

extern "C" int ob_profile_read(int fam, double* total_ms, long long* count) {
  if (fam < 0 || fam >= OB_PF_NFAM) return ob_fail("profile_read: bad fam");
  ProfFam& f = g_prof.fam[fam];
  for (int i = 0; i < ProfFam::RING; i++) prof_drain_slot(f, i);
  *total_ms = f.total_ms;
  *count = f.count;
  return 0;
}

static std::atomic<int> g_det{-1};
static int64_t g_layers_created = 0;

extern "C" int ob_deterministic(void) {
  static const bool env_on = ob_env_flag("OB_DETERMINISTIC", false);
  const int v = g_det.load(std::memory_order_relaxed);
  return v < 0 ? (env_on ? 1 : 0) : v;
}

extern "C" int ob_set_deterministic(int on) {
  if (g_layers_created > 0)
    return ob_fail(
        "set_deterministic: a layer has already been created in this "
        "process; set the mode before the first layer");
  g_det.store(on != 0 ? 1 : 0, std::memory_order_relaxed);
  return 0;
}

static int ws_ensure(float** buf, int64_t* cur, int64_t need) {
  if (need <= *cur) return 0;
  if (*buf) OB_HIP(hipFree(*buf));
  *buf = nullptr;
  *cur = 0;
  OB_HIP(hipMalloc(buf, need * sizeof(float)));
  *cur = need;
  return 0;
}


struct ob_layer {
  ob_layer_desc d;
  int B;
  float* params = nullptr;
  float* grads = nullptr;
  ob_layer_plan plan;
  float* stash = nullptr;
  int64_t* ids = nullptr;
  __bf16* shadows = nullptr;
  float p_embd = 0.f, p_resid = 0.f, p_attn = 0.f;
  int32_t layer_id = 0;
  uint64_t seed = 0;
  bool training = true;
  uint64_t next_tick = 0;
  std::vector<uint8_t> slot_drop;
  std::vector<uint64_t> slot_tick;
};

static bool has_dropout(const ob_layer* l) {
  return l->p_embd > 0.f || l->p_resid > 0.f || l->p_attn > 0.f;
}
static ob_drop_key drop_key(const ob_layer* l, int slot, int site, float p) {
  return ob_drop_make_key(l->seed, l->layer_id, site, l->slot_tick[slot], p);
}

template <class T>
static T* st_at(const ob_layer* l, int slot, int region) {
  return reinterpret_cast<T*>(l->stash + (int64_t)slot * l->plan.slot_stride +
                              l->plan.st_off[region]);
}
static __bf16* shadow(const ob_layer* l, int which) {
  return l->shadows + l->plan.sh_off[which];
}
static int64_t* slot_ids(const ob_layer* l, int slot) {
  return l->ids + (int64_t)slot * l->d.max_batch * l->d.seq_len;
}
template <class T>
struct BlockStash {
  T *x, *ln1, *qkv, *P, *am, *hmid, *ln2, *u, *gact;
  float *mean1, *rstd1, *mean2, *rstd2;
  float* lseP;
  BlockStash(const ob_layer* l, int s)
      : x(st_at<T>(l, s, ST_X)), ln1(st_at<T>(l, s, ST_LN1)),
        qkv(st_at<T>(l, s, ST_QKV)), P(st_at<T>(l, s, ST_P)),
        am(st_at<T>(l, s, ST_ATTNM)), hmid(st_at<T>(l, s, ST_HMID)),
        ln2(st_at<T>(l, s, ST_LN2)), u(st_at<T>(l, s, ST_U)),
        gact(st_at<T>(l, s, ST_G)), mean1(st_at<float>(l, s, ST_MEAN1)),
        rstd1(st_at<float>(l, s, ST_RSTD1)),
        mean2(st_at<float>(l, s, ST_MEAN2)),
        rstd2(st_at<float>(l, s, ST_RSTD2)), lseP(st_at<float>(l, s, ST_P)) {}
};
template <class T>
struct FinalStash {
  T *x, *lnf, *logits;
  float *mean, *rstd, *lse;
  int64_t* labs;
  FinalStash(const ob_layer* l, int s)
      : x(st_at<T>(l, s, ST_X)), lnf(st_at<T>(l, s, ST_LN1)),
        logits(st_at<T>(l, s, ST_LOGITS)), mean(st_at<float>(l, s, ST_MEAN1)),
        rstd(st_at<float>(l, s, ST_RSTD1)), lse(st_at<float>(l, s, ST_LSE)),
        labs(slot_ids(l, s)) {}
};
template <class T>
struct BwdWs {
  T *DY4, *DLN, *DATT, *DQKV, *DP, *pd, *dm1, *dm2;
  T *QT, *KT, *dOT;
  float* D;
  explicit BwdWs(const ob_layer* l)
      : DY4(ws<T>(WS_DY4)), DLN(ws<T>(WS_DLN)), DATT(ws<T>(WS_DATT)),
        DQKV(ws<T>(WS_DQKV)), DP(ws<T>(WS_DP)), pd(ws<T>(WS_PD_BWD)),
        dm1(ws<T>(WS_DM_ATTN)), dm2(ws<T>(WS_DM_MLP)),
        QT(ws<T>(WS_FLASH_BWD) + l->plan.pk_qt),
        KT(ws<T>(WS_FLASH_BWD) + l->plan.pk_kt),
        dOT(ws<T>(WS_FLASH_BWD) + l->plan.pk_dot),
        D(ws<float>(WS_FLASH_BWD) + l->plan.pk_d) {}
};

static bool flash_tr() {
  static const bool on = ob_env_flag("OB_FLASH_TR", true);
  return on;
}
static bool no_blaslt() {
  static const bool on = ob_env_flag("OB_NO_BLASLT", false);
  return on;
}

static ob_layer_modes process_modes() {
  static const bool fl = ob_env_flag("OB_BF16_FLASH", true),
                    drop = ob_env_flag("OB_FLASH_DROP", true),
                    hd128 = ob_env_flag("OB_FLASH_HD128", true);
  return {ob_deterministic() != 0, fl, flash_tr(), drop, hd128};
}
static ob_layer_modes modes_of_bits(int bits) {
  if (bits < 0) return process_modes();
  return {(bits & 1) != 0, (bits & 2) != 0, (bits & 4) != 0, (bits & 8) != 0,
          (bits & 16) != 0};
}

extern "C" int ob_flash_eligible(const ob_layer_desc* d, float attn_pdrop) {
  return d && ob_layer_plan_of(*d, 0.f, attn_pdrop, process_modes()).flash;
}

extern "C" int ob_layer_plan_query(const ob_layer_desc* d,
                                   const ob_dropout_desc* drop, int modes,
                                   int64_t* out, int cap) {
  if (!d || (!out && cap > 0)) return -1;
  const ob_layer_plan p =
      ob_layer_plan_of(*d, drop ? drop->resid_pdrop : 0.f,
                       drop ? drop->attn_pdrop : 0.f, modes_of_bits(modes));
  if (p.error) return ob_fail("plan_query: %s", p.error), -1;
  int64_t f[OB_LAYER_PLAN_FIELDS];
  ob_layer_plan_fields(p, f);
  for (int i = 0; i < OB_LAYER_PLAN_FIELDS && i < cap; i++) out[i] = f[i];
  return OB_LAYER_PLAN_FIELDS;
}

struct BlockParams {
  int64_t ln1_w, ln1_b, w_qkv, b_qkv, w_attnproj, b_attnproj, ln2_w, ln2_b,
      w_fc, b_fc, w_mlpproj, b_mlpproj, total;
};
static BlockParams block_params(int64_t H) {
  BlockParams p;
  int64_t o = 0;
  p.ln1_w = o; o += H;
  p.ln1_b = o; o += H;
  p.w_qkv = o; o += H * 3 * H;
  p.b_qkv = o; o += 3 * H;
  p.w_attnproj = o; o += H * H;
  p.b_attnproj = o; o += H;
  p.ln2_w = o; o += H;
  p.ln2_b = o; o += H;
  p.w_fc = o; o += H * 4 * H;
  p.b_fc = o; o += 4 * H;
  p.w_mlpproj = o; o += 4 * H * H;
  p.b_mlpproj = o; o += H;
  p.total = o;
  return p;
}

extern "C" int64_t ob_layer_param_count(const ob_layer_desc* d) {
  const int64_t H = d->n_embd, V = d->vocab_size, P = d->n_positions;
  switch (d->kind) {
    case OB_KIND_EMBED: return V * H + P * H;
    case OB_KIND_BLOCK: return block_params(H).total;
    case OB_KIND_FINAL: return 2 * H + V * H;
  }
  return -1;
}

static void ob_layer_lt_list(const ob_layer_desc* d, bool resid_drop,
                             std::vector<ob_lt_shape>* out);

struct layer_deleter {
  void operator()(ob_layer* l) const { ob_layer_destroy(l); }
};

static int layer_create(const ob_layer_desc* d, const ob_dropout_desc* drop,
                        ob_layer_t* out) {
  if (!d || !out) return ob_fail("create: null arg");
  if (d->kind < 0 || d->kind > 2) return ob_fail("create: bad kind");
  if (d->seq_len > 2048)
    return ob_fail("create: seq_len > 2048 unsupported in round 1");
  if (d->n_slots < 1) return ob_fail("create: n_slots < 1");
  const bool det = ob_deterministic() != 0;
  if (det && d->dtype != 1)
    return ob_fail(
        "create: fp32 layers (dtype 0) are not supported in deterministic "
        "mode (OB_DETERMINISTIC=1 / ob_set_deterministic): their kernels "
        "still sum with atomics");
  if (drop) {
    if (!ob_drop_p_ok(drop->embd_pdrop) || !ob_drop_p_ok(drop->resid_pdrop) ||
        !ob_drop_p_ok(drop->attn_pdrop))
      return ob_fail("create_ex: dropout probabilities must be in [0,1)");
    if (drop->layer_id < 0 || drop->layer_id >= (1 << 24))
      return ob_fail("create_ex: layer_id out of range");
  }
  std::unique_ptr<ob_layer, layer_deleter> guard(new ob_layer());
  ob_layer* const l = guard.get();
  l->d = *d;
  l->B = d->max_batch;
  l->slot_drop.assign(d->n_slots, 0);
  l->slot_tick.assign(d->n_slots, 0);
  if (drop) {
    if (d->kind == OB_KIND_EMBED) l->p_embd = drop->embd_pdrop;
    if (d->kind == OB_KIND_BLOCK) {
      l->p_resid = drop->resid_pdrop;
      l->p_attn = drop->attn_pdrop;
    }
    l->layer_id = drop->layer_id;
    l->seed = drop->seed;
  }
  const ob_layer_plan& pl = l->plan =
      ob_layer_plan_of(*d, l->p_resid, l->p_attn, process_modes());
  if (pl.error) return ob_fail("create: %s", pl.error);
  if (pl.slot_stride > 0 &&
      hipMalloc(&l->stash, (size_t)pl.slot_stride * d->n_slots *
                               sizeof(float)) != hipSuccess)
    return ob_fail("create: stash hipMalloc of %lld floats failed",
                   (long long)(pl.slot_stride * d->n_slots));
  if (pl.ids_count > 0 &&
      hipMalloc(&l->ids, (size_t)pl.ids_count * sizeof(int64_t)) !=
          hipSuccess)
    return ob_fail("create: ids hipMalloc failed");
  if (pl.shadow_count > 0) {
    if (hipMalloc(&l->shadows, (size_t)pl.shadow_count * sizeof(__bf16)) !=
        hipSuccess)
      return ob_fail("create: shadow hipMalloc failed");
    OB_HIP(hipMemset(l->shadows, 0, (size_t)pl.shadow_count * sizeof(__bf16)));
  }
  for (int i = 0; i < WS_N; i++)
    if (ws_ensure(&g_ws.buf[i], &g_ws.size[i], pl.ws[i])) return 1;
  if (pl.side && side_init()) return 1;
  if (!no_blaslt()) {
    std::vector<ob_lt_shape> shapes;
    ob_layer_lt_list(d, l->p_resid > 0.f, &shapes);
    for (const ob_lt_shape& s : shapes)
      if (ob_lt_tune_shape(s)) return 1;
  }
  g_layers_created++;
  *out = guard.release();
  return 0;
}

extern "C" int ob_layer_create(const ob_layer_desc* d, ob_layer_t* out) {
  return layer_create(d, nullptr, out);
}

extern "C" int ob_layer_create_ex(const ob_layer_desc* d,
                                  const ob_dropout_desc* drop,
                                  ob_layer_t* out) {
  return layer_create(d, drop, out);
}

extern "C" int ob_layer_uses_flash(ob_layer_t l) {
  return l && l->plan.flash ? 1 : 0;
}

extern "C" int ob_layer_set_training(ob_layer_t l, int on) {
  if (!l) return ob_fail("set_training: null layer");
  l->training = on != 0;
  return 0;
}

extern "C" int ob_layer_set_dropout_tick(ob_layer_t l, uint64_t tick) {
  if (!l) return ob_fail("set_dropout_tick: null layer");
  l->next_tick = tick;
  return 0;
}

extern "C" int ob_layer_bind(ob_layer_t l, void* params, void* grads) {
  if (!l) return ob_fail("bind: null layer");
  l->params = (float*)params;
  l->grads = (float*)grads;
  return 0;
}

extern "C" int ob_layer_set_batch(ob_layer_t l, int32_t batch) {
  if (!l) return ob_fail("set_batch: null layer");
  if (batch < 1 || batch > l->d.max_batch)
    return ob_fail("set_batch: %d out of range (max %d)", batch,
                   l->d.max_batch);
  l->B = batch;
  return 0;
}

extern "C" int ob_layer_destroy(ob_layer_t l) {
  if (!l) return 0;
  if (l->stash) hipFree(l->stash);
  if (l->ids) hipFree(l->ids);
  if (l->shadows) hipFree(l->shadows);
  delete l;
  return 0;
}

extern "C" int ob_layer_refresh_weights(ob_layer_t l, void* stream) {
  if (!l) return ob_fail("refresh: null layer");
  if (l->d.dtype != 1) return 0;
  if (!l->params) return ob_fail("refresh: params not bound");
  const int64_t H = l->d.n_embd, V = l->d.vocab_size;
  const float* p = l->params;
  switch (l->d.kind) {
    case OB_KIND_EMBED:
      return 0;
    case OB_KIND_BLOCK: {
      const BlockParams bp = block_params(H);
      if (ob_f32_to_bf16(p + bp.w_qkv, shadow(l, SH_QKV), 3 * H * H, stream) ||
          ob_f32_to_bf16_t_ld(p + bp.w_qkv, shadow(l, SH_QKV_T), H, 3 * H, H,
                              stream) ||
          ob_f32_to_bf16(p + bp.w_attnproj, shadow(l, SH_AP), H * H, stream) ||
          ob_f32_to_bf16_t_ld(p + bp.w_attnproj, shadow(l, SH_AP_T), H, H, H,
                              stream) ||
          ob_f32_to_bf16(p + bp.w_fc, shadow(l, SH_FC), 4 * H * H, stream) ||
          ob_f32_to_bf16_t_ld(p + bp.w_fc, shadow(l, SH_FC_T), H, 4 * H, H,
                              stream) ||
          ob_f32_to_bf16(p + bp.w_mlpproj, shadow(l, SH_MP), 4 * H * H,
                         stream) ||
          ob_f32_to_bf16_t_ld(p + bp.w_mlpproj, shadow(l, SH_MP_T), 4 * H, H,
                              4 * H, stream))
        return 1;
      return 0;
    }
    case OB_KIND_FINAL:
      if (ob_f32_to_bf16(p + 2 * H, shadow(l, SH_LM), V * H, stream) ||
          ob_f32_to_bf16_t_ld(p + 2 * H, shadow(l, SH_LM_T), V, H,
                              l->plan.v_pad, stream))
        return 1;
      return 0;
  }
  return ob_fail("refresh: bad kind");
}

static int gemm(int tA, int tB, int64_t M, int64_t N, int64_t K, float alpha,
                const float* A, int64_t lda, int64_t sA1, int64_t sA2,
                const float* B, int64_t ldb, int64_t sB1, int64_t sB2,
                float beta, float* C, int64_t ldc, int64_t sC1, int64_t sC2,
                int64_t n1, int64_t n2, const float* bias, const float* R,
                int atomic, int splitk, void* stream) {
  if (!no_blaslt() && !bias && !R && !atomic && splitk <= 1 && n1 == 1 &&
      n2 == 1 && M * N >= 512 * 512) {
    const int r = ob_gemm_lt_f32(tA, tB, M, N, K, alpha, A, lda, B, ldb,
                                 beta, C, ldc, stream);
    if (r >= 0) return r;
  }
  return ob_gemm_f32(tA, tB, M, N, K, alpha, A, lda, sA1, sA2, B, ldb, sB1,
                     sB2, beta, C, ldc, sC1, sC2, n1, n2, bias, R, atomic,
                     splitk, stream);
}

static int pick_splitk(int64_t M, int64_t N, int64_t K) {
  const int64_t tiles = ((M + 127) / 128) * ((N + 127) / 128);
  int sk = 1;
  while (sk < 16 && tiles * sk < 512 && (K / (sk * 2)) >= 256) sk *= 2;
  return sk;
}

static int gemm_dx_splitk(int tB, int64_t M, int64_t N, int64_t K,
                          float alpha, const float* A, int64_t lda,
                          const float* B, int64_t ldb, float* C, int64_t ldc,
                          void* stream) {
  if (!no_blaslt()) {
    const int r = ob_gemm_lt_f32(0, tB, M, N, K, alpha, A, lda, B, ldb, 0.f,
                                 C, ldc, stream);
    if (r >= 0) return r;
  }
  const int64_t tiles = ((M + 127) / 128) * ((N + 127) / 128);
  int sk = 1;
  while (sk < 16 && tiles * sk < 1024 && (K / (sk * 2)) >= 512) sk *= 2;
  if (sk == 1)
    return ob_gemm_f32(0, tB, M, N, K, alpha, A, lda, 0, 0, B, ldb, 0, 0,
                       0.f, C, ldc, 0, 0, 1, 1, nullptr, nullptr, 0, 1,
                       stream);
  OB_HIP(hipMemsetAsync(C, 0, (size_t)M * ldc * sizeof(float), S(stream)));
  return ob_gemm_f32(0, tB, M, N, K, alpha, A, lda, 0, 0, B, ldb, 0, 0, 0.f,
                     C, ldc, 0, 0, 1, 1, nullptr, nullptr, 1, sk, stream);
}


static int block_forward(ob_layer* l, int slot, const float* in, float* out,
                         void* stream) {
  const int64_t Sq = l->d.seq_len, H = l->d.n_embd, nh = l->d.n_head;
  const int64_t B = l->B, BS = B * Sq;
  const int64_t hd = H / nh;
  const float* p = l->params;
  const BlockStash<float> s(l, slot);
  const BlockParams bp = block_params(H);
  const bool dA = l->slot_drop[slot] && l->p_attn > 0.f;
  const bool dR = l->slot_drop[slot] && l->p_resid > 0.f;

  OB_HIP(hipMemcpyAsync(s.x, in, BS * H * sizeof(float),
                        hipMemcpyDeviceToDevice, S(stream)));
  if (ob_layernorm_fwd_f32(s.x, p + bp.ln1_w, p + bp.ln1_b, s.ln1, s.mean1,
                           s.rstd1, BS, H, 1e-5f, stream))
    return 1;
  if (gemm(0, 0, BS, 3 * H, H, 1.f, s.ln1, H, 0, 0, p + bp.w_qkv, 3 * H, 0, 0,
           0.f, s.qkv, 3 * H, 0, 0, 1, 1, p + bp.b_qkv, nullptr, 0, 1, stream))
    return 1;
  if (gemm(0, 1, Sq, Sq, hd, 1.f,
           s.qkv, 3 * H, Sq * 3 * H, hd,
           s.qkv + H, 3 * H, Sq * 3 * H, hd,
           0.f, s.P, Sq, nh * Sq * Sq, Sq * Sq, B, nh, nullptr, nullptr, 0, 1,
           stream))
    return 1;
  if (ob_softmax_causal_fwd_f32(s.P, B * nh, Sq, 1.f / sqrtf((float)hd),
                                stream))
    return 1;
  const float* Pv = s.P;
  if (dA) {
    if (ob_drop_scale(drop_key(l, slot, OB_DROP_ATTN, l->p_attn), 0, s.P,
                      ws<float>(WS_PD_FWD), B * nh * Sq * Sq, stream))
      return 1;
    Pv = ws<float>(WS_PD_FWD);
  }
  if (gemm(0, 0, Sq, hd, Sq, 1.f, Pv, Sq, nh * Sq * Sq, Sq * Sq, s.qkv + 2 * H,
           3 * H, Sq * 3 * H, hd, 0.f, s.am, H, Sq * H, hd, B, nh, nullptr,
           nullptr, 0, 1, stream))
    return 1;
  if (gemm(0, 0, BS, H, H, 1.f, s.am, H, 0, 0, p + bp.w_attnproj, H, 0, 0, 0.f,
           s.hmid, H, 0, 0, 1, 1, p + bp.b_attnproj, dR ? nullptr : s.x, 0, 1,
           stream))
    return 1;
  if (dR && ob_drop_add(drop_key(l, slot, OB_DROP_RESID_ATTN, l->p_resid), 0,
                        s.hmid, s.x, s.hmid, BS * H, stream))
    return 1;
  if (ob_layernorm_fwd_f32(s.hmid, p + bp.ln2_w, p + bp.ln2_b, s.ln2, s.mean2,
                           s.rstd2, BS, H, 1e-5f, stream))
    return 1;
  if (gemm(0, 0, BS, 4 * H, H, 1.f, s.ln2, H, 0, 0, p + bp.w_fc, 4 * H, 0, 0,
           0.f, s.u, 4 * H, 0, 0, 1, 1, p + bp.b_fc, nullptr, 0, 1, stream))
    return 1;
  if (ob_gelu_fwd_f32(s.u, s.gact, BS * 4 * H, stream)) return 1;
  if (gemm(0, 0, BS, H, 4 * H, 1.f, s.gact, 4 * H, 0, 0, p + bp.w_mlpproj, H, 0,
           0, 0.f, out, H, 0, 0, 1, 1, p + bp.b_mlpproj, dR ? nullptr : s.hmid,
           0, 1, stream))
    return 1;
  if (dR && ob_drop_add(drop_key(l, slot, OB_DROP_RESID_MLP, l->p_resid), 0,
                        out, s.hmid, out, BS * H, stream))
    return 1;
  return 0;
}

static int final_forward(ob_layer* l, int slot, const float* in, float* out,
                         const int64_t* labels, void* stream) {
  const int64_t Sq = l->d.seq_len, H = l->d.n_embd, V = l->d.vocab_size;
  const int64_t B = l->B, BS = B * Sq;
  const float* p = l->params;
  const FinalStash<float> s(l, slot);
  if (!labels) return ob_fail("final_forward: labels required");

  OB_HIP(hipMemcpyAsync(s.x, in, BS * H * sizeof(float),
                        hipMemcpyDeviceToDevice, S(stream)));
  OB_HIP(hipMemcpyAsync(s.labs, labels, BS * sizeof(int64_t),
                        hipMemcpyDeviceToDevice, S(stream)));
  if (ob_layernorm_fwd_f32(s.x, p + 0, p + H, s.lnf, s.mean, s.rstd, BS, H,
                           1e-5f, stream))
    return 1;
  if (gemm(0, 1, BS, V, H, 1.f, s.lnf, H, 0, 0, p + 2 * H, H, 0, 0, 0.f,
           s.logits, V, 0, 0, 1, 1, nullptr, nullptr, 0, 1, stream))
    return 1;
  OB_HIP(hipMemsetAsync(out, 0, sizeof(float), S(stream)));
  return ob_ce_fwd_f32(s.logits, s.labs, s.lse, out, B, Sq, V, stream);
}


enum {
  LG_QKV = 0, LG_AP, LG_FC, LG_MP,
  LG_DX_MP, LG_DX_FC, LG_DX_AP, LG_DX_QKV,
  LG_DW_MP, LG_DW_FC, LG_DW_AP, LG_DW_QKV,
  LG_BLOCK_N
};
enum { LG_LM = 0, LG_DLNOUT, LG_DW_LM, LG_FINAL_N };

static void block_gemms(int64_t H, int64_t BS, bool res, ob_lt_shape* g) {
  g[LG_QKV] = ob_lt_linear(BS, H, 3 * H, true, false);
  g[LG_AP] = ob_lt_linear(BS, H, H, true, res);
  g[LG_FC] = ob_lt_linear(BS, H, 4 * H, true, false);
  g[LG_MP] = ob_lt_linear(BS, 4 * H, H, true, res);
  g[LG_DX_MP] = ob_lt_linear(BS, H, 4 * H, false, false);
  g[LG_DX_FC] = ob_lt_linear(BS, 4 * H, H, false, false);
  g[LG_DX_AP] = ob_lt_linear(BS, H, H, false, false);
  g[LG_DX_QKV] = ob_lt_linear(BS, 3 * H, H, false, false);
  g[LG_DW_MP] = ob_lt_dw(4 * H, H, BS, 4 * H);
  g[LG_DW_FC] = ob_lt_dw(H, 4 * H, BS, H);
  g[LG_DW_AP] = ob_lt_dw(H, H, BS, H);
  g[LG_DW_QKV] = ob_lt_dw(H, 3 * H, BS, H);
}

static void final_gemms(int64_t H, int64_t V, int64_t v_pad, int64_t BS,
                        ob_lt_shape* g) {
  g[LG_LM] = ob_lt_linear(BS, H, v_pad, false, false);
  g[LG_DLNOUT] = ob_lt_linear(BS, v_pad, H, false, false);
  g[LG_DW_LM] = ob_lt_dw(V, H, BS, v_pad);
}

static bool lt_routed(const ob_lt_shape& s) {
  if (s.tA) return true;
  const ob_gemm_env env = {false, false, false, nullptr};
  return ob_gemm_bf16_pick(0, 1, s.M, s.N, s.K, 1, 1, BF_OUT_BF16, 1, 0.f,
                           true, env)
      .try_lt_first;
}

static void ob_layer_lt_list(const ob_layer_desc* d, bool resid_drop,
                             std::vector<ob_lt_shape>* out) {
  if (d->dtype != 1) return;
  const int64_t H = d->n_embd, V = d->vocab_size;
  const int64_t BS = (int64_t)d->max_batch * d->seq_len;
  ob_lt_shape g[LG_BLOCK_N];
  int n = 0;
  if (d->kind == OB_KIND_BLOCK) {
    block_gemms(H, BS, true, g);
    n = LG_BLOCK_N;
  } else if (d->kind == OB_KIND_FINAL) {
    final_gemms(H, V, ob_v_pad(V), BS, g);
    n = LG_FINAL_N;
  }
  for (int i = 0; i < n; i++)
    if (lt_routed(g[i])) out->push_back(g[i]);
  if (d->kind == OB_KIND_BLOCK && resid_drop) {
    block_gemms(H, BS, false, g);
    for (int i : {LG_AP, LG_MP})
      if (lt_routed(g[i])) out->push_back(g[i]);
  }
}

extern "C" int ob_layer_lt_shapes(const ob_layer_desc* d, int64_t* out,
                                  int cap) {
  if (!d || (!out && cap > 0)) return -1;
  std::vector<ob_lt_shape> v;
  ob_layer_lt_list(d, false, &v);
  for (int i = 0; i < (int)v.size() && i < cap; i++) {
    const ob_lt_shape& s = v[i];
    int64_t* o = out + (int64_t)i * OB_LT_SHAPE_FIELDS;
    o[0] = s.tA, o[1] = s.tB, o[2] = s.M, o[3] = s.N, o[4] = s.K;
    o[5] = s.lda, o[6] = s.ldb, o[7] = s.ldc, o[8] = s.c_f32, o[9] = s.beta1;
    o[10] = s.bias, o[11] = s.cin, o[12] = s.ab_f32;
  }
  return (int)v.size();
}

static int linear_bf(const ob_lt_shape& s, const void* in, const void* W,
                     const float* bias, const void* res, void* out,
                     void* stream) {
  if ((bias != nullptr) != (s.bias != 0) || (res != nullptr) != (s.cin != 0))
    return ob_fail("linear_bf: operands do not match the listed shape");
  ob_bf16_gemm g;
  g.A = in, g.B = W, g.C = out, g.bias = bias, g.residual = res;
  g.M = s.M, g.N = s.N, g.K = s.K, g.lda = s.lda, g.ldb = s.ldb;
  g.ldc = s.ldc, g.stream = stream;
  return ob_gemm_bf16_run(g);
}

static ob_bf16_gemm attn_gemm(int tA, int tB, int64_t M, int64_t N, int64_t K,
                              float alpha, int64_t B, int64_t nh,
                              void* stream) {
  ob_bf16_gemm g;
  g.transA = tA, g.transB = tB, g.M = M, g.N = N, g.K = K, g.alpha = alpha;
  g.n1 = B, g.n2 = nh, g.stream = stream;
  return g;
}

static int dw_bf16_ws(const ob_lt_shape& s, const __bf16* act,
                      const __bf16* dY, float* gout, void* stream) {
  const int64_t actw = s.M, dyw = s.N, BS = s.K, ldc = s.ldc;
  if (!no_blaslt()) {
    const int r = ob_gemm_lt(s.tA, s.tB, s.M, s.N, s.K, 1.f, act, s.lda, dY,
                             s.ldb, 1.f, gout, s.ldc, s.c_f32, stream);
    if (r >= 0) return r;
  }
  ob_bf16_gemm g;
  g.C = gout, g.M = actw, g.N = dyw, g.K = BS, g.ldc = ldc;
  g.out_kind = 2, g.stream = stream;
  g.splitk = ob_deterministic() ? 1 : pick_splitk(actw, dyw, BS);
  if ((actw % 128) || (dyw % 128) || (BS % 128)) {
    g.transA = 1, g.transB = 0;
    g.A = act, g.lda = actw, g.B = dY, g.ldb = dyw;
    return ob_gemm_bf16_run(g);
  }
  __bf16* XT = ws<__bf16>(WS_DW_A);
  __bf16* DYT = ws<__bf16>(WS_DW_B);
  if (ob_transpose_bf16(act, XT, BS, actw, stream)) return 1;
  if (ob_transpose_bf16(dY, DYT, BS, dyw, stream)) return 1;
  g.A = XT, g.lda = BS, g.B = DYT, g.ldb = BS;
  return ob_gemm_bf16_run(g);
}

static int block_forward_bf16(ob_layer* l, int slot, const __bf16* in,
                              __bf16* out, void* stream) {
  const int64_t Sq = l->d.seq_len, H = l->d.n_embd, nh = l->d.n_head;
  const int64_t B = l->B, BS = B * Sq;
  const int64_t hd = H / nh;
  const float* p = l->params;
  const BlockStash<__bf16> s(l, slot);
  const BlockParams bp = block_params(H);
  const bool dA = l->slot_drop[slot] && l->p_attn > 0.f;
  const bool dR = l->slot_drop[slot] && l->p_resid > 0.f;
  ob_lt_shape lg[LG_BLOCK_N];
  block_gemms(H, BS, !dR, lg);

  if (OB_PROF(OB_PF_LN, stream,
              ob_layernorm_fwd_copy_bf16(in, p + bp.ln1_w, p + bp.ln1_b, s.ln1,
                                         s.x, s.mean1, s.rstd1, BS, H, 1e-5f,
                                         stream)))
    return 1;
  if (OB_PROF(OB_PF_GEMM_FWD, stream,
              linear_bf(lg[LG_QKV], s.ln1, shadow(l, SH_QKV_T), p + bp.b_qkv,
                        nullptr, s.qkv, stream)))
    return 1;
  if (l->plan.flash && flash_tr()) {
    if (dA) {
      if (OB_PROF(OB_PF_FLASH_FWD, stream,
                  ob_flash_fwd_nt_drop_bf16(s.qkv, s.am, s.lseP, B, Sq, H, nh,
                                            1.f / sqrtf((float)hd), l->seed,
                                            l->layer_id, l->slot_tick[slot],
                                            l->p_attn, stream)))
        return 1;
    } else if (OB_PROF(OB_PF_FLASH_FWD, stream,
                       ob_flash_fwd_nt_bf16(s.qkv, s.am, s.lseP, B, Sq, H, nh,
                                            1.f / sqrtf((float)hd), stream)))
      return 1;
  } else if (l->plan.flash) {
    __bf16* VTw = ws<__bf16>(WS_FLASH_VT);
    if (OB_PROF(OB_PF_FLASH_FWD, stream,
                ob_transpose_bf16_b(s.qkv + 2 * H, VTw, Sq, 64, Sq * 3 * H, 64,
                                    3 * H, B, nh, stream)))
      return 1;
    if (OB_PROF(OB_PF_FLASH_FWD, stream,
                ob_flash_fwd_bf16(s.qkv, VTw, s.am, s.lseP, B, Sq, H, nh,
                                  1.f / sqrtf((float)hd), stream)))
      return 1;
  } else {
    ob_bf16_gemm qk = attn_gemm(0, 1, Sq, Sq, hd, 1.f, B, nh, stream);
    qk.A = s.qkv, qk.lda = 3 * H, qk.sA1 = Sq * 3 * H, qk.sA2 = hd;
    qk.B = s.qkv + H, qk.ldb = 3 * H, qk.sB1 = Sq * 3 * H, qk.sB2 = hd;
    qk.C = s.P, qk.ldc = Sq, qk.sC1 = nh * Sq * Sq, qk.sC2 = Sq * Sq;
    if (OB_PROF(OB_PF_ATTN_MAT, stream, ob_gemm_bf16_run(qk))) return 1;
    if (OB_PROF(OB_PF_ATTN_MAT, stream,
                ob_softmax_causal_fwd_bf16(s.P, B * nh, Sq,
                                           1.f / sqrtf((float)hd), stream)))
      return 1;
    const __bf16* Pv = s.P;
    if (dA) {
      if (OB_PROF(OB_PF_ELEM, stream,
                  ob_drop_scale(drop_key(l, slot, OB_DROP_ATTN, l->p_attn), 1,
                                s.P, ws<__bf16>(WS_PD_FWD), B * nh * Sq * Sq,
                                stream)))
        return 1;
      Pv = ws<__bf16>(WS_PD_FWD);
    }
    ob_bf16_gemm pv = attn_gemm(0, 0, Sq, hd, Sq, 1.f, B, nh, stream);
    pv.A = Pv, pv.lda = Sq, pv.sA1 = nh * Sq * Sq, pv.sA2 = Sq * Sq;
    pv.B = s.qkv + 2 * H, pv.ldb = 3 * H, pv.sB1 = Sq * 3 * H, pv.sB2 = hd;
    pv.C = s.am, pv.ldc = H, pv.sC1 = Sq * H, pv.sC2 = hd;
    if (OB_PROF(OB_PF_ATTN_MAT, stream, ob_gemm_bf16_run(pv))) return 1;
  }
  if (OB_PROF(OB_PF_GEMM_FWD, stream,
              linear_bf(lg[LG_AP], s.am, shadow(l, SH_AP_T), p + bp.b_attnproj,
                        dR ? nullptr : s.x, s.hmid, stream)))
    return 1;
  if (dR &&
      OB_PROF(OB_PF_ELEM, stream,
              ob_drop_add(drop_key(l, slot, OB_DROP_RESID_ATTN, l->p_resid), 1,
                          s.hmid, s.x, s.hmid, BS * H, stream)))
    return 1;
  if (OB_PROF(OB_PF_LN, stream,
              ob_layernorm_fwd_bf16(s.hmid, p + bp.ln2_w, p + bp.ln2_b, s.ln2,
                                    s.mean2, s.rstd2, BS, H, 1e-5f, stream)))
    return 1;
  if (OB_PROF(OB_PF_FC_FWD, stream,
              linear_bf(lg[LG_FC], s.ln2, shadow(l, SH_FC_T), p + bp.b_fc,
                        nullptr, s.u, stream)))
    return 1;
  if (OB_PROF(OB_PF_ELEM, stream,
              ob_gelu_fwd_bf16(s.u, s.gact, BS * 4 * H, stream)))
    return 1;
  if (OB_PROF(OB_PF_GEMM_FWD, stream,
              linear_bf(lg[LG_MP], s.gact, shadow(l, SH_MP_T),
                        p + bp.b_mlpproj, dR ? nullptr : s.hmid, out, stream)))
    return 1;
  if (dR &&
      OB_PROF(OB_PF_ELEM, stream,
              ob_drop_add(drop_key(l, slot, OB_DROP_RESID_MLP, l->p_resid), 1,
                          out, s.hmid, out, BS * H, stream)))
    return 1;
  return 0;
}

static int final_forward_bf16(ob_layer* l, int slot, const __bf16* in,
                              float* out, const int64_t* labels,
                              void* stream) {
  const int64_t Sq = l->d.seq_len, H = l->d.n_embd, V = l->d.vocab_size;
  const int64_t B = l->B, BS = B * Sq;
  const float* p = l->params;
  const FinalStash<__bf16> s(l, slot);
  if (!labels) return ob_fail("final_forward_bf16: labels required");
  ob_lt_shape lg[LG_FINAL_N];
  final_gemms(H, V, l->plan.v_pad, BS, lg);

  OB_HIP(hipMemcpyAsync(s.labs, labels, BS * sizeof(int64_t),
                        hipMemcpyDeviceToDevice, S(stream)));
  if (OB_PROF(OB_PF_LN, stream,
              ob_layernorm_fwd_copy_bf16(in, p + 0, p + H, s.lnf, s.x, s.mean,
                                         s.rstd, BS, H, 1e-5f, stream)))
    return 1;
  if (OB_PROF(OB_PF_GEMM_FWD, stream,
              linear_bf(lg[LG_LM], s.lnf, shadow(l, SH_LM), nullptr, nullptr,
                        s.logits, stream)))
    return 1;
  OB_HIP(hipMemsetAsync(out, 0, sizeof(float), S(stream)));
  float* const wsf = ob_deterministic() ? ws<float>(WS_DET_FWD) : nullptr;
  return OB_PROF(OB_PF_CE, stream,
                 ob_ce_fwd_ws(s.logits, s.labs, s.lse, out, B, Sq, V,
                              l->plan.v_pad, wsf, stream));
}

static int block_backward_bf16(ob_layer* l, int slot, const __bf16* dout,
                               __bf16* din, void* stream) {
  const int64_t Sq = l->d.seq_len, H = l->d.n_embd, nh = l->d.n_head;
  const int64_t B = l->B, BS = B * Sq;
  const int64_t hd = H / nh;
  const float scale = 1.f / sqrtf((float)hd);
  const float* p = l->params;
  const BlockStash<__bf16> s(l, slot);
  const BwdWs<__bf16> w(l);
  float* g = l->grads;
  const BlockParams bp = block_params(H);
  const bool dA = l->slot_drop[slot] && l->p_attn > 0.f;
  const bool dR = l->slot_drop[slot] && l->p_resid > 0.f;
  ob_lt_shape lg[LG_BLOCK_N];
  block_gemms(H, BS, !dR, lg);
  const bool det = ob_deterministic() != 0;
  float* const wsm = det ? ws<float>(WS_DET_MAIN) : nullptr;

  void* const side = (void*)g_side.stream;
  OB_SIDE_FENCE(S(stream), g_side.stream);

  const __bf16* dmlp = dout;
  if (dR) {
    if (OB_PROF(OB_PF_ELEM, stream,
                ob_drop_scale_colsum(
                    drop_key(l, slot, OB_DROP_RESID_MLP, l->p_resid), 1, dout,
                    w.dm2, g + bp.b_mlpproj, BS, H, stream, wsm)))
      return 1;
    dmlp = w.dm2;
    OB_SIDE_FENCE(S(stream), g_side.stream);
  }
  if (OB_PROF(OB_PF_GEMM_DX, stream,
              linear_bf(lg[LG_DX_MP], dmlp, shadow(l, SH_MP), nullptr, nullptr,
                        w.DY4, stream)))
    return 1;
  if (OB_PROF(OB_PF_GEMM_DW, side,
              dw_bf16_ws(lg[LG_DW_MP], s.gact, dmlp, g + bp.w_mlpproj, side)))
    return 1;
  if (OB_PROF(OB_PF_ELEM, stream,
              ob_gelu_bwd_colsum_ws(s.u, w.DY4, w.DY4, g + bp.b_fc, BS, 4 * H,
                                    wsm, stream)))
    return 1;
  OB_SIDE_FENCE(S(stream), g_side.stream);
  if (OB_PROF(OB_PF_GEMM_DW, side,
              dw_bf16_ws(lg[LG_DW_FC], s.ln2, w.DY4, g + bp.w_fc, side)))
    return 1;
  if (OB_PROF(OB_PF_GEMM_DX, stream,
              linear_bf(lg[LG_DX_FC], w.DY4, shadow(l, SH_FC), nullptr,
                        nullptr, w.DLN, stream)))
    return 1;
  if (OB_PROF(OB_PF_LN, stream,
              ob_layernorm_bwd_res_ws(s.hmid, p + bp.ln2_w, s.mean2, s.rstd2,
                                      w.DLN, dout, din, g + bp.ln2_w,
                                      g + bp.ln2_b,
                                      dR ? nullptr : g + bp.b_mlpproj,
                                      dR ? nullptr : g + bp.b_attnproj,
                                      BS, H, wsm, stream)))
    return 1;
  const __bf16* dap = din;
  if (dR) {
    if (OB_PROF(OB_PF_ELEM, stream,
                ob_drop_scale_colsum(
                    drop_key(l, slot, OB_DROP_RESID_ATTN, l->p_resid), 1, din,
                    w.dm1, g + bp.b_attnproj, BS, H, stream, wsm)))
      return 1;
    dap = w.dm1;
  }
  OB_SIDE_FENCE(S(stream), g_side.stream);
  if (OB_PROF(OB_PF_GEMM_DX, stream,
              linear_bf(lg[LG_DX_AP], dap, shadow(l, SH_AP), nullptr, nullptr,
                        w.DATT, stream)))
    return 1;
  if (OB_PROF(OB_PF_GEMM_DW, side,
              dw_bf16_ws(lg[LG_DW_AP], s.am, dap, g + bp.w_attnproj, side)))
    return 1;
  hipEvent_t ev_din_done = side_evt();
  OB_HIP(hipEventRecord(ev_din_done, g_side.stream));
  const bool flash_nt = l->plan.flash && flash_tr();
  if (flash_nt) {
    float* const dbq = det ? nullptr : g + bp.b_qkv;
    if (dA) {
      if (OB_PROF(OB_PF_FLASH_BWD, stream,
                  ob_flash_bwd_nt_d_drop_bf16(s.qkv, s.am, w.DATT, s.lseP, w.D,
                                              w.DQKV, dbq, B, Sq, H, nh, scale,
                                              l->seed, l->layer_id,
                                              l->slot_tick[slot], l->p_attn,
                                              stream)))
        return 1;
    } else if (OB_PROF(OB_PF_FLASH_BWD, stream,
                       ob_flash_bwd_nt_d_bf16(s.qkv, s.am, w.DATT, s.lseP, w.D,
                                              w.DQKV, dbq, B, Sq, H, nh, scale,
                                              stream)))
      return 1;
  } else if (l->plan.flash) {
    if (OB_PROF(OB_PF_FLASH_BWD, stream,
                ob_transpose_bf16_b(s.qkv, w.QT, Sq, 64, Sq * 3 * H, 64, 3 * H,
                                    B, nh, stream)))
      return 1;
    if (OB_PROF(OB_PF_FLASH_BWD, stream,
                ob_transpose_bf16_b(s.qkv + H, w.KT, Sq, 64, Sq * 3 * H, 64,
                                    3 * H, B, nh, stream)))
      return 1;
    if (OB_PROF(OB_PF_FLASH_BWD, stream,
                ob_transpose_bf16_b(w.DATT, w.dOT, Sq, 64, Sq * H, 64, H, B,
                                    nh, stream)))
      return 1;
    if (OB_PROF(OB_PF_FLASH_BWD, stream,
                ob_flash_dsum_bf16(s.am, w.DATT, w.D, B, Sq, H, nh, stream)))
      return 1;
    if (OB_PROF(OB_PF_FLASH_BWD, stream,
                ob_flash_bwd_bf16(s.qkv, w.QT, w.KT, w.dOT, w.DATT, s.lseP,
                                  w.D, w.DQKV, B, Sq, H, nh, scale, stream)))
      return 1;
  } else {
    ob_bf16_gemm dp = attn_gemm(0, 1, Sq, Sq, hd, 1.f, B, nh, stream);
    dp.A = w.DATT, dp.lda = H, dp.sA1 = Sq * H, dp.sA2 = hd;
    dp.B = s.qkv + 2 * H, dp.ldb = 3 * H, dp.sB1 = Sq * 3 * H, dp.sB2 = hd;
    dp.C = w.DP, dp.ldc = Sq, dp.sC1 = nh * Sq * Sq, dp.sC2 = Sq * Sq;
    if (OB_PROF(OB_PF_ATTN_MAT, stream, ob_gemm_bf16_run(dp))) return 1;
    const __bf16* Pv = s.P;
    if (dA) {
      const ob_drop_key ka = drop_key(l, slot, OB_DROP_ATTN, l->p_attn);
      if (OB_PROF(OB_PF_ELEM, stream,
                  ob_drop_scale(ka, 1, s.P, w.pd, B * nh * Sq * Sq, stream)))
        return 1;
      if (OB_PROF(OB_PF_ELEM, stream,
                  ob_drop_scale(ka, 1, w.DP, w.DP, B * nh * Sq * Sq, stream)))
        return 1;
      Pv = w.pd;
    }
    if (OB_PROF(OB_PF_ATTN_MAT, stream,
                ob_softmax_causal_bwd_bf16(s.P, w.DP, B * nh, Sq, stream)))
      return 1;
    ob_bf16_gemm dq = attn_gemm(0, 0, Sq, hd, Sq, scale, B, nh, stream);
    dq.A = w.DP, dq.lda = Sq, dq.sA1 = nh * Sq * Sq, dq.sA2 = Sq * Sq;
    dq.B = s.qkv + H, dq.ldb = 3 * H, dq.sB1 = Sq * 3 * H, dq.sB2 = hd;
    dq.C = w.DQKV, dq.ldc = 3 * H, dq.sC1 = Sq * 3 * H, dq.sC2 = hd;
    if (OB_PROF(OB_PF_ATTN_MAT, stream, ob_gemm_bf16_run(dq))) return 1;
    ob_bf16_gemm dk = dq;
    dk.transA = 1, dk.B = s.qkv, dk.C = w.DQKV + H;
    if (OB_PROF(OB_PF_ATTN_MAT, stream, ob_gemm_bf16_run(dk))) return 1;
    ob_bf16_gemm dv = dk;
    dv.alpha = 1.f, dv.A = Pv, dv.C = w.DQKV + 2 * H;
    dv.B = w.DATT, dv.ldb = H, dv.sB1 = Sq * H, dv.sB2 = hd;
    if (OB_PROF(OB_PF_ATTN_MAT, stream, ob_gemm_bf16_run(dv))) return 1;
  }
  OB_SIDE_FENCE(S(stream), g_side.stream);
  if ((!flash_nt || det) &&
      OB_PROF(OB_PF_ELEM, side,
              ob_colsum_ws(w.DQKV, g + bp.b_qkv, BS, 3 * H,
                           det ? ws<float>(WS_DET_SIDE) : nullptr, side)))
    return 1;
  if (OB_PROF(OB_PF_GEMM_DW, side,
              dw_bf16_ws(lg[LG_DW_QKV], s.ln1, w.DQKV, g + bp.w_qkv, side)))
    return 1;
  if (OB_PROF(OB_PF_GEMM_DX, stream,
              linear_bf(lg[LG_DX_QKV], w.DQKV, shadow(l, SH_QKV), nullptr,
                        nullptr, w.DLN, stream)))
    return 1;
  OB_HIP(hipStreamWaitEvent(S(stream), ev_din_done, 0));
  if (OB_PROF(OB_PF_LN, stream,
              ob_layernorm_bwd_ws(s.x, p + bp.ln1_w, s.mean1, s.rstd1, w.DLN,
                                  din, g + bp.ln1_w, g + bp.ln1_b, BS, H, 1,
                                  wsm, stream)))
    return 1;
  OB_SIDE_FENCE(g_side.stream, S(stream));
  return 0;
}

static int final_backward_bf16(ob_layer* l, int slot, const float* dout,
                               __bf16* din, void* stream) {
  const int64_t Sq = l->d.seq_len, H = l->d.n_embd, V = l->d.vocab_size;
  const int64_t B = l->B, BS = B * Sq;
  const float* p = l->params;
  const FinalStash<__bf16> s(l, slot);
  const BwdWs<__bf16> w(l);
  float* g = l->grads;
  ob_lt_shape lg[LG_FINAL_N];
  final_gemms(H, V, l->plan.v_pad, BS, lg);
  const ob_lt_shape& dwlm = lg[LG_DW_LM];

  if (OB_PROF(OB_PF_CE, stream,
              ob_ce_bwd_bf16(s.logits, s.labs, s.lse, dout, B, Sq, V,
                             l->plan.v_pad, stream)))
    return 1;
  {
    OB_SIDE_FENCE(S(stream), g_side.stream);
    void* const side = (void*)g_side.stream;
    int r = -1;
    if (!no_blaslt())
      r = OB_PROF(OB_PF_GEMM_DW, side,
                  ob_gemm_lt(dwlm.tA, dwlm.tB, dwlm.M, dwlm.N, dwlm.K, 1.f,
                             s.logits, dwlm.lda, s.lnf, dwlm.ldb, 1.f,
                             g + 2 * H, dwlm.ldc, dwlm.c_f32, side));
    if (r > 0) return 1;
    if (r < 0) {
      __bf16* DLT = ws<__bf16>(WS_DW_A);
      __bf16* LNT = ws<__bf16>(WS_DW_B);
      if (ob_transpose_bf16(s.logits, DLT, BS, l->plan.v_pad, side)) return 1;
      if (ob_transpose_bf16(s.lnf, LNT, BS, H, side)) return 1;
      ob_bf16_gemm dw;
      dw.A = DLT, dw.lda = BS, dw.B = LNT, dw.ldb = BS;
      dw.C = g + 2 * H, dw.ldc = H, dw.M = l->plan.v_pad, dw.N = H, dw.K = BS;
      dw.out_kind = 2, dw.splitk = ob_deterministic() ? 1 : 2, dw.Mr = V;
      dw.stream = side;
      if (OB_PROF(OB_PF_GEMM_DW, side, ob_gemm_bf16_nt_dispatch(dw)))
        return 1;
    }
  }
  if (OB_PROF(OB_PF_GEMM_DX, stream,
              linear_bf(lg[LG_DLNOUT], s.logits, shadow(l, SH_LM_T),
                        nullptr, nullptr, w.DLN, stream)))
    return 1;
  float* const wsm = ob_deterministic() ? ws<float>(WS_DET_MAIN) : nullptr;
  if (OB_PROF(OB_PF_LN, stream,
              ob_layernorm_bwd_ws(s.x, p + 0, s.mean, s.rstd, w.DLN, din,
                                  g + 0, g + H, BS, H, 0, wsm, stream)))
    return 1;
  OB_SIDE_FENCE(g_side.stream, S(stream));
  return 0;
}

extern "C" int ob_layer_forward(ob_layer_t l, int32_t slot, const void* in,
                                void* out, const int64_t* labels,
                                void* stream) {
  if (!l) return ob_fail("forward: null layer");
  if (!l->params) return ob_fail("forward: params not bound");
  if (slot < 0 || slot >= l->d.n_slots) return ob_fail("forward: bad slot");
  const bool drop = l->training && has_dropout(l);
  l->slot_drop[slot] = drop ? 1 : 0;
  l->slot_tick[slot] = l->next_tick;
  if (drop) l->next_tick++;
  switch (l->d.kind) {
    case OB_KIND_EMBED: {
      const int64_t Sq = l->d.seq_len, H = l->d.n_embd, V = l->d.vocab_size;
      const int64_t BS = (int64_t)l->B * Sq;
      int64_t* ids = slot_ids(l, slot);
      OB_HIP(hipMemcpyAsync(ids, in, BS * sizeof(int64_t),
                            hipMemcpyDeviceToDevice, S(stream)));
      if (drop)
        return OB_PROF(OB_PF_ELEM, stream,
                       ob_embed_fwd_drop(
                           drop_key(l, slot, OB_DROP_EMBD, l->p_embd),
                           l->d.dtype == 1, ids, l->params, l->params + V * H,
                           out, l->B, Sq, H, stream));
      if (l->d.dtype == 1)
        return OB_PROF(OB_PF_ELEM, stream,
                       ob_embed_fwd_bf16(ids, l->params, l->params + V * H,
                                         out, l->B, Sq, H, stream));
      return OB_PROF(OB_PF_ELEM, stream,
                     ob_embed_fwd_f32(ids, l->params, l->params + V * H,
                                      (float*)out, l->B, Sq, H, stream));
    }
    case OB_KIND_BLOCK:
      if (l->d.dtype == 1)
        return block_forward_bf16(l, slot, (const __bf16*)in, (__bf16*)out,
                                  stream);
      return block_forward(l, slot, (const float*)in, (float*)out, stream);
    case OB_KIND_FINAL:
      if (l->d.dtype == 1)
        return final_forward_bf16(l, slot, (const __bf16*)in, (float*)out,
                                  labels, stream);
      return final_forward(l, slot, (const float*)in, (float*)out, labels,
                           stream);
  }
  return ob_fail("forward: bad kind");
}


static int block_backward(ob_layer* l, int slot, const float* dout, float* din,
                          void* stream) {
  const int64_t Sq = l->d.seq_len, H = l->d.n_embd, nh = l->d.n_head;
  const int64_t B = l->B, BS = B * Sq;
  const int64_t hd = H / nh;
  const float scale = 1.f / sqrtf((float)hd);
  const float* p = l->params;
  const BlockStash<float> s(l, slot);
  const BwdWs<float> w(l);
  float* g = l->grads;
  const BlockParams bp = block_params(H);
  const bool dA = l->slot_drop[slot] && l->p_attn > 0.f;
  const bool dR = l->slot_drop[slot] && l->p_resid > 0.f;

  OB_HIP(hipMemcpyAsync(din, dout, BS * H * sizeof(float),
                        hipMemcpyDeviceToDevice, S(stream)));
  const float* dmlp = dout;
  if (dR) {
    if (ob_drop_scale_colsum(drop_key(l, slot, OB_DROP_RESID_MLP, l->p_resid),
                             0, dout, w.dm2, g + bp.b_mlpproj, BS, H, stream))
      return 1;
    dmlp = w.dm2;
  }
  if (gemm(0, 1, BS, 4 * H, H, 1.f, dmlp, H, 0, 0, p + bp.w_mlpproj, H, 0, 0,
           0.f, w.DY4, 4 * H, 0, 0, 1, 1, nullptr, nullptr, 0, 1, stream))
    return 1;
  if (gemm(1, 0, 4 * H, H, BS, 1.f, s.gact, 4 * H, 0, 0, dmlp, H, 0, 0, 1.f,
           g + bp.w_mlpproj, H, 0, 0, 1, 1, nullptr, nullptr, 1,
           pick_splitk(4 * H, H, BS), stream))
    return 1;
  if (!dR && ob_colsum_f32(dout, g + bp.b_mlpproj, BS, H, stream)) return 1;
  if (ob_gelu_bwd_f32(s.u, w.DY4, w.DY4, BS * 4 * H, stream)) return 1;
  if (gemm(1, 0, H, 4 * H, BS, 1.f, s.ln2, H, 0, 0, w.DY4, 4 * H, 0, 0, 1.f,
           g + bp.w_fc, 4 * H, 0, 0, 1, 1, nullptr, nullptr, 1,
           pick_splitk(H, 4 * H, BS), stream))
    return 1;
  if (ob_colsum_f32(w.DY4, g + bp.b_fc, BS, 4 * H, stream)) return 1;
  if (gemm_dx_splitk(1, BS, H, 4 * H, 1.f, w.DY4, 4 * H, p + bp.w_fc, 4 * H,
                     w.DLN, H, stream))
    return 1;
  if (ob_layernorm_bwd_f32(s.hmid, p + bp.ln2_w, s.mean2, s.rstd2, w.DLN, din,
                           g + bp.ln2_w, g + bp.ln2_b, BS, H, 1, stream))
    return 1;
  const float* dap = din;
  if (dR) {
    if (ob_drop_scale_colsum(drop_key(l, slot, OB_DROP_RESID_ATTN, l->p_resid),
                             0, din, w.dm1, g + bp.b_attnproj, BS, H, stream))
      return 1;
    dap = w.dm1;
  }
  if (gemm_dx_splitk(1, BS, H, H, 1.f, dap, H, p + bp.w_attnproj, H, w.DATT,
                     H, stream))
    return 1;
  if (gemm(1, 0, H, H, BS, 1.f, s.am, H, 0, 0, dap, H, 0, 0, 1.f,
           g + bp.w_attnproj, H, 0, 0, 1, 1, nullptr, nullptr, 1,
           pick_splitk(H, H, BS), stream))
    return 1;
  if (!dR && ob_colsum_f32(din, g + bp.b_attnproj, BS, H, stream)) return 1;
  if (gemm(0, 1, Sq, Sq, hd, 1.f, w.DATT, H, Sq * H, hd, s.qkv + 2 * H, 3 * H,
           Sq * 3 * H, hd, 0.f, w.DP, Sq, nh * Sq * Sq, Sq * Sq, B, nh, nullptr,
           nullptr, 0, 1, stream))
    return 1;
  const float* Pv = s.P;
  if (dA) {
    const ob_drop_key ka = drop_key(l, slot, OB_DROP_ATTN, l->p_attn);
    if (ob_drop_scale(ka, 0, s.P, w.pd, B * nh * Sq * Sq, stream)) return 1;
    if (ob_drop_scale(ka, 0, w.DP, w.DP, B * nh * Sq * Sq, stream)) return 1;
    Pv = w.pd;
  }
  if (ob_softmax_causal_bwd_f32(s.P, w.DP, B * nh, Sq, stream)) return 1;
  if (gemm(0, 0, Sq, hd, Sq, scale, w.DP, Sq, nh * Sq * Sq, Sq * Sq, s.qkv + H,
           3 * H, Sq * 3 * H, hd, 0.f, w.DQKV, 3 * H, Sq * 3 * H, hd, B, nh,
           nullptr, nullptr, 0, 1, stream))
    return 1;
  if (gemm(1, 0, Sq, hd, Sq, scale, w.DP, Sq, nh * Sq * Sq, Sq * Sq, s.qkv,
           3 * H, Sq * 3 * H, hd, 0.f, w.DQKV + H, 3 * H, Sq * 3 * H, hd, B, nh,
           nullptr, nullptr, 0, 1, stream))
    return 1;
  if (gemm(1, 0, Sq, hd, Sq, 1.f, Pv, Sq, nh * Sq * Sq, Sq * Sq, w.DATT, H,
           Sq * H, hd, 0.f, w.DQKV + 2 * H, 3 * H, Sq * 3 * H, hd, B, nh,
           nullptr, nullptr, 0, 1, stream))
    return 1;
  if (ob_colsum_f32(w.DQKV, g + bp.b_qkv, BS, 3 * H, stream)) return 1;
  if (gemm(1, 0, H, 3 * H, BS, 1.f, s.ln1, H, 0, 0, w.DQKV, 3 * H, 0, 0, 1.f,
           g + bp.w_qkv, 3 * H, 0, 0, 1, 1, nullptr, nullptr, 1,
           pick_splitk(H, 3 * H, BS), stream))
    return 1;
  if (gemm_dx_splitk(1, BS, H, 3 * H, 1.f, w.DQKV, 3 * H, p + bp.w_qkv, 3 * H,
                     w.DLN, H, stream))
    return 1;
  return ob_layernorm_bwd_f32(s.x, p + bp.ln1_w, s.mean1, s.rstd1, w.DLN, din,
                              g + bp.ln1_w, g + bp.ln1_b, BS, H, 1, stream);
}

static int final_backward(ob_layer* l, int slot, const float* dout, float* din,
                          void* stream) {
  const int64_t Sq = l->d.seq_len, H = l->d.n_embd, V = l->d.vocab_size;
  const int64_t B = l->B, BS = B * Sq;
  const float* p = l->params;
  const FinalStash<float> s(l, slot);
  const BwdWs<float> w(l);
  float* g = l->grads;

  if (ob_ce_bwd_f32(s.logits, s.labs, s.lse, (const float*)dout, B, Sq, V,
                    stream))
    return 1;
  if (gemm(1, 0, V, H, BS, 1.f, s.logits, V, 0, 0, s.lnf, H, 0, 0, 1.f,
           g + 2 * H, H, 0, 0, 1, 1, nullptr, nullptr, 1, 1, stream))
    return 1;
  if (gemm_dx_splitk(0, BS, H, V, 1.f, s.logits, V, p + 2 * H, H, w.DLN, H,
                     stream))
    return 1;
  return ob_layernorm_bwd_f32(s.x, p + 0, s.mean, s.rstd, w.DLN, din, g + 0,
                              g + H, BS, H, 0, stream);
}

extern "C" int ob_layer_backward(ob_layer_t l, int32_t slot, const void* dout,
                                 void* din, void* stream) {
  if (!l) return ob_fail("backward: null layer");
  if (!l->params || !l->grads) return ob_fail("backward: buffers not bound");
  if (slot < 0 || slot >= l->d.n_slots) return ob_fail("backward: bad slot");
  switch (l->d.kind) {
    case OB_KIND_EMBED: {
      const int64_t Sq = l->d.seq_len, H = l->d.n_embd, V = l->d.vocab_size;
      int64_t* ids = slot_ids(l, slot);
      if (ob_deterministic()) {
        const ob_drop_key ke = drop_key(l, slot, OB_DROP_EMBD, l->p_embd);
        return OB_PROF(OB_PF_ELEM, stream,
                       ob_embed_bwd_det(l->slot_drop[slot] ? &ke : nullptr,
                                        ids, dout, l->grads, l->grads + V * H,
                                        l->B, Sq, H, stream));
      }
      if (l->slot_drop[slot])
        return OB_PROF(OB_PF_ELEM, stream,
                       ob_embed_bwd_drop(
                           drop_key(l, slot, OB_DROP_EMBD, l->p_embd),
                           l->d.dtype == 1, ids, dout, l->grads,
                           l->grads + V * H, l->B, Sq, H, stream));
      if (l->d.dtype == 1)
        return OB_PROF(OB_PF_ELEM, stream,
                       ob_embed_bwd_bf16(ids, dout, l->grads,
                                         l->grads + V * H, l->B, Sq, H,
                                         stream));
      return OB_PROF(OB_PF_ELEM, stream,
                     ob_embed_bwd_f32(ids, (const float*)dout, l->grads,
                                      l->grads + V * H, l->B, Sq, H,
                                      stream));
    }
    case OB_KIND_BLOCK:
      if (!dout || !din) return ob_fail("block backward: dout/din required");
      if (l->d.dtype == 1)
        return block_backward_bf16(l, slot, (const __bf16*)dout, (__bf16*)din,
                                   stream);
      return block_backward(l, slot, (const float*)dout, (float*)din, stream);
    case OB_KIND_FINAL:
      if (!din) return ob_fail("final backward: din required");
      if (l->d.dtype == 1)
        return final_backward_bf16(l, slot, (const float*)dout, (__bf16*)din,
                                   stream);
      return final_backward(l, slot, (const float*)dout, (float*)din, stream);
  }
  return ob_fail("backward: bad kind");
}
```

Before: 754,100 tokens/s.

## Add tuned split-K batched weight-gradient GEMM with slab fold kernel

Weight-gradient GEMMs with few output tiles but a very long K can now run as a strided-batched hipBLASLt matmul over K slices into a float scratch slab. A fold kernel then sums the slices into the fp32 gradient. The autotuner times the sliced candidates alongside the plain algorithms and records a slice count per shape. The goal is to fill idle compute units when the output tile count is below the CU count, at the cost of extra slab traffic, a fold launch and longer tuning.

Measured after the change: 769,800 tokens/s (median of 6 runs). 1.02x the previous value.

```diff
diff --git a/include/oobleck_stage.h b/include/oobleck_stage.h
--- a/include/oobleck_stage.h
+++ b/include/oobleck_stage.h
@@ -172,6 +172,16 @@
 int64_t ob_gemm_lt_table_size(void);
 int64_t ob_gemm_lt_untuned_uses(void);
 int ob_gemm_lt_plan_index(const int64_t* shape, void* stream);
+
+int ob_dw_slices_admit(const int64_t* shape, int s, int cus,
+                       int64_t slab_floats);
+int ob_gemm_lt_dw_sliced(int64_t M, int64_t N, int64_t K, const void* A,
+                         int64_t lda, const void* B, int64_t ldb, void* C,
+                         int64_t ldc, int s, void* slab, int64_t slab_floats,
+                         void* stream, int32_t* used);
+int ob_gemm_lt_tune_slab(const int64_t* shape, int64_t slab_floats);
+int ob_gemm_lt_slices(const int64_t* shape, double* out, int32_t* slices,
+                      int32_t* index, double* us, int cap);
 
 int ob_flash_fwd_nt_bf16(const void* qkv, void* O, void* lse, int64_t B,
                          int64_t Sq, int64_t H, int64_t nh, float scale,
diff --git a/oobleck_amd/_ext.py b/oobleck_amd/_ext.py
--- a/oobleck_amd/_ext.py
+++ b/oobleck_amd/_ext.py
@@ -148,6 +148,14 @@
     lib.ob_gemm_lt_untuned_uses.argtypes = []
     lib.ob_gemm_lt_untuned_uses.restype = i64
     lib.ob_gemm_lt_plan_index.argtypes = [shape, vp]
+    lib.ob_dw_slices_admit.argtypes = [shape, i32, i32, i64]
+    lib.ob_gemm_lt_dw_sliced.argtypes = [i64, i64, i64, vp, i64, vp, i64, vp,
+                                         i64, i32, vp, i64, vp,
+                                         ctypes.POINTER(i32)]
+    lib.ob_gemm_lt_tune_slab.argtypes = [shape, i64]
+    lib.ob_gemm_lt_slices.argtypes = [shape, ctypes.POINTER(ctypes.c_double),
+                                      ctypes.POINTER(i32), ctypes.POINTER(i32),
+                                      ctypes.POINTER(ctypes.c_double), i32]
     lib.ob_profile_enable.argtypes = [i32]
     lib.ob_profile_enable.restype = None
     lib.ob_profile_reset.argtypes = []
@@ -261,6 +269,25 @@
             for i in range(max(0, min(n, cap)))]
 
 
+def dw_slices_admit(shape, s: int, cus: int, slab_floats: int) -> bool:
+    return bool(get_ext().ob_dw_slices_admit(lt_shape(*shape), s, cus,
+                                             slab_floats))
+
+
+def lt_slices(shape, cap: int = 32) -> dict | None:
+    out = (ctypes.c_double * 6)()
+    sl, idx = (ctypes.c_int32 * cap)(), (ctypes.c_int32 * cap)()
+    us = (ctypes.c_double * cap)()
+    n = get_ext().ob_gemm_lt_slices(lt_shape(*shape), out, sl, idx, us, cap)
+    if n < 0 or not out[0]:
+        return None
+    return {"slices": int(out[1]), "slice_index": int(out[2]),
+            "us_sliced": out[3], "added_ms": out[4],
+            "fastest_slices": int(out[5]),
+            "pairs": [{"slices": sl[i], "index": idx[i], "us": us[i]}
+                      for i in range(min(n, cap))]}
+
+
 PLAN_STASH = ("x", "mean1", "rstd1", "ln1", "qkv", "p", "attnm", "hmid",
               "mean2", "rstd2", "ln2", "u", "g", "logits", "lse")
 PLAN_SHADOWS = ("qkv", "qkv_t", "ap", "ap_t", "fc", "fc_t", "mp", "mp_t",
diff --git a/oobleck_amd/build.py b/oobleck_amd/build.py
--- a/oobleck_amd/build.py
+++ b/oobleck_amd/build.py
@@ -21,6 +21,7 @@
            PKG_DIR / "csrc" / "ob_flash_common.h",
            PKG_DIR / "csrc" / "ob_bf16.h",
            PKG_DIR / "csrc" / "ob_gemm_route.h",
+           PKG_DIR / "csrc" / "ob_dw_slices.h",
            PKG_DIR / "csrc" / "ob_philox.h"]
 
 
diff --git a/oobleck_amd/csrc/ob_blaslt.hip b/oobleck_amd/csrc/ob_blaslt.hip
--- a/oobleck_amd/csrc/ob_blaslt.hip
+++ b/oobleck_amd/csrc/ob_blaslt.hip
@@ -1,4 +1,5 @@
 #include "ob_internal.h"
+#include "ob_dw_slices.h"
 
 #include <hipblaslt/hipblaslt-ext.hpp>
 #include <hipblaslt/hipblaslt.h>
@@ -13,6 +14,8 @@
 #include <set>
 #include <string>
 #include <tuple>
+#include <type_traits>
+#include <utility>
 #include <vector>
 
 namespace {
@@ -21,9 +24,10 @@
 
 struct Key {
   ob_lt_shape s;
+  int batch = 1;
   auto tie() const {
     return std::tie(s.tA, s.tB, s.M, s.N, s.K, s.lda, s.ldb, s.ldc, s.c_f32,
-                    s.beta1, s.bias, s.cin, s.ab_f32);
+                    s.beta1, s.bias, s.cin, s.ab_f32, batch);
   }
   bool operator<(const Key& o) const { return tie() < o.tie(); }
 };
@@ -39,6 +43,7 @@
   int index = -1;
   bool ok = false;
   bool untuned = false;
+  int slices = 1;
 };
 
 struct LtCtx {
@@ -62,6 +67,14 @@
     double us;
   };
   std::vector<Timed> timed;
+  int slices = 1, slice_index = -1;
+  double us_sliced = 0;
+  double slice_ms = 0;
+  struct Sliced {
+    int slices, index, pos;
+    double us;
+  };
+  std::vector<Sliced> sliced;
 };
 std::mutex g_tab_mu;
 std::map<Key, LtChoice> g_tab;
@@ -81,7 +94,10 @@
   return &g_lt_by_stream.emplace(stream, ctx).first->second;
 }
 
-void lt_problem_create(const ob_lt_shape& k, const void* bias, LtProblem* p) {
+void lt_problem_create(const ob_lt_shape& k0, const void* bias, LtProblem* p,
+                       int batch = 1) {
+  ob_lt_shape k = k0;
+  if (batch > 1) k.K = k0.K / batch, k.ldc = k0.N;
   const hipblasOperation_t opA = k.tB ? HIPBLAS_OP_T : HIPBLAS_OP_N;
   const hipblasOperation_t opB = k.tA ? HIPBLAS_OP_T : HIPBLAS_OP_N;
   const int64_t a_rows = k.tB ? k.K : k.N, a_cols = k.tB ? k.N : k.K;
@@ -106,6 +122,19 @@
   hipblasLtMatrixLayoutCreate(&p->lb, abt, b_rows, b_cols, k.lda);
   hipblasLtMatrixLayoutCreate(&p->lc, k.c_f32 ? HIP_R_32F : HIP_R_16BF, k.N,
                               k.M, k.ldc);
+  if (batch > 1) {
+    const int32_t n = batch;
+    const int64_t sa = k.K * k.ldb, sb = k.K * k.lda, sc = k.M * k.N;
+    const std::pair<hipblasLtMatrixLayout_t, int64_t> ls[] = {
+        {p->la, sa}, {p->lb, sb}, {p->lc, sc}};
+    for (const auto& l : ls) {
+      hipblasLtMatrixLayoutSetAttribute(
+          l.first, HIPBLASLT_MATRIX_LAYOUT_BATCH_COUNT, &n, sizeof(n));
+      hipblasLtMatrixLayoutSetAttribute(
+          l.first, HIPBLASLT_MATRIX_LAYOUT_STRIDED_BATCH_OFFSET, &l.second,
+          sizeof(l.second));
+    }
+  }
 }
 
 void lt_problem_destroy(LtProblem* p) {
@@ -131,14 +160,13 @@
 }
 
 bool lt_algo_from_index(hipblasLtHandle_t h, const LtProblem& p,
-                        const ob_lt_shape& k, int index,
-                        hipblasLtMatmulAlgo_t* algo) {
+                        float beta, int index, hipblasLtMatmulAlgo_t* algo) {
   std::vector<int> idx{index};
   std::vector<hipblasLtMatmulHeuristicResult_t> r;
   if (hipblaslt_ext::getAlgosFromIndex(h, idx, r) != HIPBLAS_STATUS_SUCCESS ||
       r.empty())
     return false;
-  const float alpha = 1.f, beta = k.beta1 ? 1.f : 0.f;
+  const float alpha = 1.f;
   size_t need = 0;
   if (hipblaslt_ext::matmulIsAlgoSupported(h, p.desc, &alpha, p.la, p.lb,
                                            &beta, p.lc, p.lc, r[0].algo,
@@ -151,17 +179,22 @@
 
 LtPlan lt_plan_build(LtCtx* ctx, const Key& key, const void* bias) {
   LtPlan p;
-  lt_problem_create(key.s, bias, &p.p);
+  lt_problem_create(key.s, bias, &p.p, key.batch);
   int index = -1;
   {
     std::lock_guard<std::mutex> lk(g_tab_mu);
-    auto it = g_tab.find(key);
-    if (it == g_tab.end())
-      p.untuned = lt_tune_on();
-    else if (it->second.tuned && lt_tune_on())
-      index = it->second.index;
-  }
-  if (index >= 0 && lt_algo_from_index(ctx->h, p.p, key.s, index, &p.algo)) {
+    auto it = g_tab.find(Key{key.s});
+    if (it == g_tab.end()) {
+      p.untuned = lt_tune_on() && key.batch == 1;
+    } else if (it->second.tuned && lt_tune_on()) {
+      if (key.batch == 1)
+        index = it->second.index, p.slices = it->second.slices;
+      else if (it->second.slices == key.batch)
+        index = it->second.slice_index;
+    }
+  }
+  const float beta = key.batch == 1 && key.s.beta1 ? 1.f : 0.f;
+  if (index >= 0 && lt_algo_from_index(ctx->h, p.p, beta, index, &p.algo)) {
     p.index = index;
     p.ok = true;
     return p;
@@ -174,6 +207,75 @@
     p.ok = true;
   }
   return p;
+}
+
+
+int dw_slices_env() {
+  static const int n = ob_env_int("OB_DW_SLICES", 0);
+  return n < 0 ? 0 : n;
+}
+
+int lt_cus() {
+  static const int n = [] {
+    int dev = 0, v = 0;
+    if (hipGetDevice(&dev) != hipSuccess ||
+        hipDeviceGetAttribute(&v, hipDeviceAttributeMultiprocessorCount,
+                              dev) != hipSuccess)
+      return 0;
+    return v;
+  }();
+  return n;
+}
+
+ob_dw_slice_shape dw_slice_shape(const ob_lt_shape& k) {
+  return {k.tA, k.tB, k.c_f32, k.beta1, !k.bias && !k.cin && !k.ab_f32,
+          k.M,  k.N,  k.K,     k.ldc};
+}
+
+}
+
+template <int S, int W>
+__global__ __launch_bounds__(256) void k_dw_fold(float* __restrict__ g,
+                                                 const float* __restrict__ slab,
+                                                 int64_t n) {
+  using V = typename std::conditional<W == 4, float4, float>::type;
+  const int64_t i = (int64_t)blockIdx.x * 256 + threadIdx.x;
+  if (i >= n / W) return;
+  V v[S];
+#pragma unroll
+  for (int k = 0; k < S; k++)
+    v[k] = reinterpret_cast<const V*>(slab + (int64_t)k * n)[i];
+  V acc = reinterpret_cast<const V*>(g)[i];
+  V t = v[0];
+#pragma unroll
+  for (int k = 1; k < S; k++) t += v[k];
+  acc += t;
+  reinterpret_cast<V*>(g)[i] = acc;
+}
+
+namespace {
+
+template <int W>
+int dw_fold_w(float* g, const float* slab, int s, int64_t n, hipStream_t st) {
+  const int64_t blocks = (n / W + 255) / 256;
+  if (blocks > INT32_MAX) return ob_fail("dw_fold: output too large");
+  const dim3 grid((unsigned)blocks);
+  switch (s) {
+    case 2: k_dw_fold<2, W><<<grid, 256, 0, st>>>(g, slab, n); break;
+    case 4: k_dw_fold<4, W><<<grid, 256, 0, st>>>(g, slab, n); break;
+    case 8: k_dw_fold<8, W><<<grid, 256, 0, st>>>(g, slab, n); break;
+    case 16: k_dw_fold<16, W><<<grid, 256, 0, st>>>(g, slab, n); break;
+    default: return ob_fail("dw_fold: %d slices", s);
+  }
+  OB_LAUNCH_CHECK();
+  return 0;
+}
+
+int dw_fold(float* g, const float* slab, int s, int64_t n, hipStream_t st) {
+  if (n <= 0) return 0;
+  const bool vec = n % 4 == 0 && (uintptr_t)g % 16 == 0 &&
+                   (uintptr_t)slab % 16 == 0;
+  return vec ? dw_fold_w<4>(g, slab, s, n, st) : dw_fold_w<1>(g, slab, s, n, st);
 }
 
 
@@ -225,13 +327,15 @@
   hipStream_t stream = nullptr;
   hipblasLtHandle_t h = nullptr;
   void *ws = nullptr, *A = nullptr, *B = nullptr, *C = nullptr, *Cref = nullptr,
-       *Cin = nullptr, *bias = nullptr;
+       *Cin = nullptr, *bias = nullptr, *slab = nullptr;
   double* acc = nullptr;
   hipEvent_t e0 = nullptr, e1 = nullptr;
   LtProblem p;
+  std::vector<LtProblem> sp;
   ~TuneScratch() {
     lt_problem_destroy(&p);
-    for (void* q : {ws, A, B, C, Cref, Cin, bias, (void*)acc})
+    for (LtProblem& q : sp) lt_problem_destroy(&q);
+    for (void* q : {ws, A, B, C, Cref, Cin, bias, slab, (void*)acc})
       if (q) (void)hipFree(q);
     if (e0) (void)hipEventDestroy(e0);
     if (e1) (void)hipEventDestroy(e1);
@@ -243,12 +347,13 @@
 struct Cand {
   hipblasLtMatmulAlgo_t algo;
   int pos = 0;
+  int slices = 1, prob = -1;
   int reps = 1;
   float warm_us = 0.f;
   std::vector<float> us;
 };
 
-bool lt_tune_run(const ob_lt_shape& k, LtChoice* out) {
+bool lt_tune_run(const ob_lt_shape& k, int64_t slab_floats, LtChoice* out) {
   const int n_env = ob_env_int("OB_LT_TUNE_N", 8);
   const int n_max = n_env < 1 ? 1 : n_env > 128 ? 128 : n_env;
   constexpr int kRounds = 5;
@@ -315,21 +420,77 @@
     }
   }
   const int nres = (int)res.size();
-  auto run = [&](hipblasLtMatmulAlgo_t& algo, void* dst) {
-    return hipblasLtMatmul(t.h, t.p.desc, &alpha, t.B, t.p.la, t.A, t.p.lb,
-                           &beta, t.Cin ? t.Cin : dst, t.p.lc, dst, t.p.lc,
-                           &algo, t.ws, kLtWs, t.stream);
-  };
-  const double bound = k.c_f32 ? 1e-3 : 1.0 / 256;
-  std::vector<Cand> cands;
+  std::vector<Cand> listed;
   for (int i = 0; i < nres; i++) {
     if (res[i].state != HIPBLAS_STATUS_SUCCESS) {
       out->dropped++;
       continue;
     }
+    Cand c;
+    c.algo = res[i].algo;
+    c.pos = i;
+    listed.push_back(c);
+  }
+  if (listed.empty() || listed[0].pos != 0 || listed[0].slices != 1)
+    return false;
+  const auto ts0 = std::chrono::steady_clock::now();
+  auto since = [](std::chrono::steady_clock::time_point a) {
+    return std::chrono::duration<double, std::milli>(
+               std::chrono::steady_clock::now() - a)
+        .count();
+  };
+  const int forced = dw_slices_env();
+  int slist[4], ns = 0;
+  if (slab_floats > 0 && forced != 1)
+    ns = ob_dw_slices_list(dw_slice_shape(k), lt_cus(), slab_floats, slist);
+  if (ns > 0) {
+    const int per_env = ob_env_int("OB_LT_TUNE_SLICE_N", 2);
+    const int per = per_env < 1 ? 1 : per_env > 8 ? 8 : per_env;
+    int smax = 0;
+    for (int j = 0; j < ns; j++) {
+      const int s = slist[j];
+      if (forced > 1 ? s != forced : s > OB_DW_SLICES_AUTO_MAX) continue;
+      t.sp.emplace_back();
+      lt_problem_create(k, nullptr, &t.sp.back(), s);
+      hipblasLtMatmulHeuristicResult_t sres[8];
+      const int got = lt_heuristic(t.h, t.sp.back(), per, sres);
+      for (int i = 0; i < got; i++) {
+        if (sres[i].state != HIPBLAS_STATUS_SUCCESS) continue;
+        Cand c;
+        c.algo = sres[i].algo;
+        c.pos = i, c.slices = s, c.prob = (int)t.sp.size() - 1;
+        listed.push_back(c);
+        smax = s;
+      }
+    }
+    if (smax) LT_TRY(hipMalloc(&t.slab, (size_t)smax * k.M * k.N * 4));
+  }
+  out->slice_ms += since(ts0);
+  const float zero = 0.f;
+  auto run = [&](Cand& c, void* dst) {
+    if (c.slices > 1) {
+      const LtProblem& q = t.sp[c.prob];
+      const hipblasStatus_t st = hipblasLtMatmul(
+          t.h, q.desc, &alpha, t.B, q.la, t.A, q.lb, &zero, t.slab, q.lc,
+          t.slab, q.lc, &c.algo, t.ws, kLtWs, t.stream);
+      if (st != HIPBLAS_STATUS_SUCCESS) return st;
+      return dw_fold((float*)dst, (const float*)t.slab, c.slices, k.M * k.N,
+                     t.stream)
+                 ? HIPBLAS_STATUS_INTERNAL_ERROR
+                 : HIPBLAS_STATUS_SUCCESS;
+    }
+    return hipblasLtMatmul(t.h, t.p.desc, &alpha, t.B, t.p.la, t.A, t.p.lb,
+                           &beta, t.Cin ? t.Cin : dst, t.p.lc, dst, t.p.lc,
+                           &c.algo, t.ws, kLtWs, t.stream);
+  };
+  const double bound = k.c_f32 ? 1e-3 : 1.0 / 256;
+  std::vector<Cand> cands;
+  for (size_t i = 0; i < listed.size(); i++) {
+    const auto tc0 = std::chrono::steady_clock::now();
+    const bool sliced = listed[i].slices > 1;
     void* dst = i == 0 ? t.Cref : t.C;
     LT_TRY(hipMemsetAsync(dst, 0, nC * es_c, t.stream));
-    const hipblasStatus_t st = run(res[i].algo, dst);
+    const hipblasStatus_t st = run(listed[i], dst);
     if (i == 0 && st != HIPBLAS_STATUS_SUCCESS) return false;
     if (st != HIPBLAS_STATUS_SUCCESS) {
       LT_TRY(hipStreamSynchronize(t.stream));
@@ -352,10 +513,8 @@
     } else {
       LT_TRY(hipStreamSynchronize(t.stream));
     }
-    Cand c;
-    c.algo = res[i].algo;
-    c.pos = i;
-    cands.push_back(c);
+    cands.push_back(listed[i]);
+    if (sliced) out->slice_ms += since(tc0);
   }
   out->tried = nres;
   enum { V_OK = 0, V_DROP = 1, V_HIP = 2 };
@@ -363,7 +522,7 @@
     if (hipEventRecord(t.e0, t.stream) != hipSuccess) return (int)V_HIP;
     bool lib_ok = true;
     for (int r = 0; r < reps && lib_ok; r++)
-      lib_ok = run(c.algo, t.C) == HIPBLAS_STATUS_SUCCESS;
+      lib_ok = run(c, t.C) == HIPBLAS_STATUS_SUCCESS;
     float ms = 0.f;
     if (hipEventRecord(t.e1, t.stream) != hipSuccess ||
         hipEventSynchronize(t.e1) != hipSuccess ||
@@ -385,25 +544,30 @@
   LT_TRY(hipMemsetAsync(t.C, 0, nC * es_c, t.stream));
   for (size_t i = 0; i < cands.size();) {
     Cand& c = cands[i];
+    const auto tc0 = std::chrono::steady_clock::now();
     float us = 0.f;
     int v = visit(c, 1, &us);
     if (v == V_OK) v = visit(c, 8, &us);
+    if (c.slices > 1) out->slice_ms += since(tc0);
     if (v == V_HIP || (v == V_DROP && !drop(i))) return false;
     if (v == V_DROP) continue;
     c.warm_us = us;
     c.reps = reps_for(us);
     i++;
   }
-  if ((int)cands.size() > n_max) {
-    std::stable_sort(cands.begin() + 1, cands.end(),
+  const int n_unsl = (int)std::count_if(
+      cands.begin(), cands.end(), [](const Cand& c) { return c.slices == 1; });
+  if (n_unsl > n_max) {
+    std::stable_sort(cands.begin() + 1, cands.begin() + n_unsl,
                      [](const Cand& a, const Cand& b) {
                        return a.warm_us < b.warm_us;
                      });
-    cands.resize(n_max);
+    cands.erase(cands.begin() + n_max, cands.begin() + n_unsl);
   }
   for (int r = 0; r < kRounds; r++)
     for (size_t i = 0; i < cands.size();) {
       Cand& c = cands[i];
+      const auto tc0 = std::chrono::steady_clock::now();
       float us = 0.f;
       int v = V_OK;
       for (int attempt = 0; attempt < 4; attempt++) {
@@ -411,6 +575,7 @@
         if (v != V_OK || us * c.reps >= 1000.f || c.reps >= 4096) break;
         c.reps = std::max(c.reps + 1, reps_for(us));
       }
+      if (c.slices > 1) out->slice_ms += since(tc0);
       if (v == V_HIP || (v == V_DROP && !drop(i))) return false;
       if (v == V_DROP) continue;
       c.us.push_back(us);
@@ -426,7 +591,7 @@
   double best_med = med0;
   out->timed.push_back(
       {hipblaslt_ext::getIndexFromAlgo(cands[0].algo), 0, med0});
-  for (size_t i = 1; i < cands.size(); i++) {
+  for (size_t i = 1; i < cands.size() && cands[i].slices == 1; i++) {
     const double m = median_of(cands[i].us);
     out->timed.push_back(
         {hipblaslt_ext::getIndexFromAlgo(cands[i].algo), cands[i].pos, m});
@@ -443,6 +608,27 @@
   out->us_chosen = best_med;
   out->index = hipblaslt_ext::getIndexFromAlgo(cands[best].algo);
   out->chosen_name = hipblaslt_ext::getKernelNameFromAlgo(t.h, cands[best].algo);
+  size_t sbest = 0;
+  double sbest_med = 0;
+  for (size_t i = 1; i < cands.size(); i++) {
+    if (cands[i].slices == 1) continue;
+    const double m = median_of(cands[i].us);
+    out->sliced.push_back({cands[i].slices,
+                           hipblaslt_ext::getIndexFromAlgo(cands[i].algo),
+                           cands[i].pos, m});
+    if (!sbest || m < sbest_med) sbest_med = m, sbest = i;
+  }
+  if (sbest) {
+    out->us_sliced = sbest_med;
+    const bool wins =
+        sbest_med < med0 - spread0 && sbest_med < best_med &&
+        *std::max_element(cands[sbest].us.begin(), cands[sbest].us.end()) <
+            min0;
+    if (wins || forced > 1) {
+      out->slices = cands[sbest].slices;
+      out->slice_index = hipblaslt_ext::getIndexFromAlgo(cands[sbest].algo);
+    }
+  }
   out->tuned = true;
   return true;
 }
@@ -459,7 +645,7 @@
 
 }
 
-int ob_lt_tune_shape(const ob_lt_shape& s) {
+int ob_lt_tune_shape(const ob_lt_shape& s, int64_t slab_floats) {
   if (!lt_tune_on()) return 0;
   if (s.M <= 0 || s.N <= 0 || s.K <= 0 || s.ldc < s.N ||
       s.lda < (s.tA ? s.M : s.K) || s.ldb < (s.tB ? s.K : s.N))
@@ -472,7 +658,7 @@
   OB_HIP(hipDeviceSynchronize());
   const auto t0 = std::chrono::steady_clock::now();
   LtChoice c;
-  if (!lt_tune_run(s, &c)) {
+  if (!lt_tune_run(s, slab_floats, &c)) {
     c.tuned = false;
     c.index = c.top1_index;
     (void)hipGetLastError();
@@ -485,13 +671,22 @@
     std::lock_guard<std::mutex> lk(g_tab_mu);
     g_tab.emplace(key, c);
   }
-  for (auto& sc : g_lt_by_stream) {
-    auto it = sc.second.plans.find(key);
-    if (it == sc.second.plans.end()) continue;
-    lt_problem_destroy(&it->second.p);
-    sc.second.plans.erase(it);
-  }
+  for (auto& sc : g_lt_by_stream)
+    for (int batch = 1; batch <= OB_DW_SLICES_MAX; batch *= 2) {
+      auto it = sc.second.plans.find(Key{s, batch});
+      if (it == sc.second.plans.end()) continue;
+      lt_problem_destroy(&it->second.p);
+      sc.second.plans.erase(it);
+    }
   return 0;
+}
+
+static const LtPlan* lt_plan_get(LtCtx* ctx, const Key& key,
+                                 const void* bias) {
+  auto it = ctx->plans.find(key);
+  if (it == ctx->plans.end())
+    it = ctx->plans.emplace(key, lt_plan_build(ctx, key, bias)).first;
+  return &it->second;
 }
 
 static int lt_matmul(int tA, int tB, int64_t M, int64_t N, int64_t K,
@@ -504,10 +699,7 @@
   if (!ctx) return ob_fail("hipblasLt per-stream context init failed");
   const Key key{ob_lt_shape_of(tA, tB, M, N, K, lda, ldb, ldc, c_f32, beta,
                                bias != nullptr, Cin != C, ab_f32)};
-  auto it = ctx->plans.find(key);
-  if (it == ctx->plans.end())
-    it = ctx->plans.emplace(key, lt_plan_build(ctx, key, bias)).first;
-  const LtPlan& p = it->second;
+  const LtPlan& p = *lt_plan_get(ctx, key, bias);
   if (!p.ok) return -1;
   if (p.untuned) g_untuned_uses.fetch_add(1, std::memory_order_relaxed);
   if (bias)
@@ -521,6 +713,67 @@
   return 0;
 }
 
+static int lt_dw_sliced(LtCtx* ctx, const ob_lt_shape& s, int n, const void* A,
+                        const void* B, float* C, float* slab, void* stream) {
+  const LtPlan& p = *lt_plan_get(ctx, Key{s, n}, nullptr);
+  if (!p.ok) return -1;
+  const float one = 1.f, zero = 0.f;
+  const hipblasStatus_t st = hipblasLtMatmul(
+      ctx->h, p.p.desc, &one, B, p.p.la, A, p.p.lb, &zero, slab, p.p.lc, slab,
+      p.p.lc, &p.algo, ctx->ws, kLtWs, reinterpret_cast<hipStream_t>(stream));
+  if (st != HIPBLAS_STATUS_SUCCESS)
+    return ob_fail("hipblasLtMatmul (sliced) failed (%d)", (int)st);
+  return dw_fold(C, slab, n, s.M * s.N, reinterpret_cast<hipStream_t>(stream));
+}
+
+int ob_lt_dw_run(const ob_lt_shape& s, const void* act, const void* dY,
+                 float* gout, float* slab, int64_t slab_floats, void* stream) {
+  LtCtx* ctx = lt_ctx(stream);
+  if (!ctx) return ob_fail("hipblasLt per-stream context init failed");
+  const int n = lt_plan_get(ctx, Key{s}, nullptr)->slices;
+  if (n > 1 && slab &&
+      ob_dw_slices_ok(dw_slice_shape(s), n, lt_cus(), slab_floats)) {
+    const int r = lt_dw_sliced(ctx, s, n, act, dY, gout, slab, stream);
+    if (r >= 0) return r;
+  }
+  return lt_matmul(s.tA, s.tB, s.M, s.N, s.K, 1.f, act, s.lda, dY, s.ldb, 1.f,
+                   gout, s.ldc, s.c_f32, nullptr, 0, stream);
+}
+
+extern "C" int ob_gemm_lt_dw_sliced(int64_t M, int64_t N, int64_t K,
+                                    const void* A, int64_t lda, const void* B,
+                                    int64_t ldb, void* C, int64_t ldc, int s,
+                                    void* slab, int64_t slab_floats,
+                                    void* stream, int32_t* used) {
+  if (!A || !B || !C) return ob_fail("gemm_lt_dw_sliced: null operand");
+  if (M <= 0 || N <= 0 || K <= 0 || lda < M || ldb < N || ldc < N)
+    return ob_fail("gemm_lt_dw_sliced: bad shape");
+  const ob_lt_shape k = ob_lt_dw(M, N, K, lda);
+  ob_lt_shape kk = k;
+  kk.ldb = ldb, kk.ldc = ldc;
+  if (used) *used = 1;
+  LtCtx* ctx = lt_ctx(stream);
+  if (!ctx) return ob_fail("hipblasLt per-stream context init failed");
+  if (slab && ob_dw_slices_ok(dw_slice_shape(kk), s, lt_cus(), slab_floats)) {
+    const int r =
+        lt_dw_sliced(ctx, kk, s, A, B, (float*)C, (float*)slab, stream);
+    if (r == 0 && used) *used = s;
+    if (r >= 0) return r;
+  }
+  const int r = lt_matmul(1, 0, M, N, K, 1.f, A, lda, B, ldb, 1.f, C, ldc, 1,
+                          nullptr, 0, stream);
+  return r < 0 ? ob_fail("gemm_lt_dw_sliced: the library has no solution") : r;
+}
+
+extern "C" int ob_dw_slices_admit(const int64_t* shape, int s, int cus,
+                                  int64_t slab_floats) {
+  if (!shape) return 0;
+  return ob_dw_slices_ok(dw_slice_shape(key_from_i64(shape).s), s, cus,
+                         slab_floats)
+             ? 1
+             : 0;
+}
+
 extern "C" int ob_gemm_lt(int tA, int tB, int64_t M, int64_t N, int64_t K,
                           float alpha, const void* A, int64_t lda,
                           const void* B, int64_t ldb, float beta, void* C,
@@ -561,6 +814,13 @@
 extern "C" int ob_gemm_lt_tune(const int64_t* shape) {
   if (!shape) return ob_fail("gemm_lt_tune: null shape");
   return ob_lt_tune_shape(key_from_i64(shape).s);
+}
+
+extern "C" int ob_gemm_lt_tune_slab(const int64_t* shape,
+                                    int64_t slab_floats) {
+  if (!shape) return ob_fail("gemm_lt_tune_slab: null shape");
+  return ob_lt_tune_shape(key_from_i64(shape).s,
+                          slab_floats > 0 ? slab_floats : 0);
 }
 
 extern "C" int ob_gemm_lt_choice(const int64_t* shape, double* out,
@@ -585,6 +845,28 @@
   return 0;
 }
 
+extern "C" int ob_gemm_lt_slices(const int64_t* shape, double* out,
+                                 int32_t* slices, int32_t* index, double* us,
+                                 int cap) {
+  if (!shape || !out || (cap > 0 && (!slices || !index || !us))) return -1;
+  for (int i = 0; i < 6; i++) out[i] = 0;
+  std::lock_guard<std::mutex> lk(g_tab_mu);
+  auto it = g_tab.find(key_from_i64(shape));
+  if (it == g_tab.end()) return 0;
+  const LtChoice& c = it->second;
+  auto v = c.sliced;
+  std::stable_sort(v.begin(), v.end(),
+                   [](const LtChoice::Sliced& a, const LtChoice::Sliced& b) {
+                     return a.us < b.us;
+                   });
+  out[0] = 1, out[1] = c.tuned ? c.slices : 1;
+  out[2] = c.tuned ? c.slice_index : -1, out[3] = c.us_sliced;
+  out[4] = c.slice_ms, out[5] = v.empty() ? 1 : v[0].slices;
+  for (int i = 0; i < (int)v.size() && i < cap; i++)
+    slices[i] = v[i].slices, index[i] = v[i].index, us[i] = v[i].us;
+  return (int)v.size();
+}
+
 extern "C" int ob_gemm_lt_candidates(const int64_t* shape, int32_t* index,
                                      int32_t* pos, double* us, int cap) {
   if (!shape || (cap > 0 && (!index || !pos || !us))) return -1;
diff --git a/oobleck_amd/csrc/ob_dw_slices.h b/oobleck_amd/csrc/ob_dw_slices.h
--- /dev/null
+++ b/oobleck_amd/csrc/ob_dw_slices.h
@@ -0,0 +1,36 @@
+#pragma once
+#include <cstdint>
+
+#define OB_DW_SLICE_TILE 128
+#define OB_DW_SLICE_K_ALIGN 256
+#define OB_DW_SLICE_K_MIN 1024
+#define OB_DW_SLICES_MAX 16
+#define OB_DW_SLICES_AUTO_MAX 2
+
+struct ob_dw_slice_shape {
+  int tA, tB, c_f32, beta1;
+  bool plain;
+  int64_t M, N, K, ldc;
+};
+
+inline bool ob_dw_slices_ok(const ob_dw_slice_shape& k, int s, int cus,
+                            int64_t slab_floats) {
+  if (!(k.tA == 1 && k.tB == 0 && k.c_f32 && k.beta1 && k.plain)) return false;
+  if (k.M <= 0 || k.N <= 0 || k.K <= 0 || k.ldc != k.N) return false;
+  if (s != 2 && s != 4 && s != 8 && s != OB_DW_SLICES_MAX) return false;
+  const int64_t tiles = ((k.M + OB_DW_SLICE_TILE - 1) / OB_DW_SLICE_TILE) *
+                        ((k.N + OB_DW_SLICE_TILE - 1) / OB_DW_SLICE_TILE);
+  if (tiles >= cus) return false;
+  if (k.K % s) return false;
+  const int64_t ks = k.K / s;
+  if (ks % OB_DW_SLICE_K_ALIGN || ks < OB_DW_SLICE_K_MIN) return false;
+  return (int64_t)s * k.M * k.N <= slab_floats;
+}
+
+inline int ob_dw_slices_list(const ob_dw_slice_shape& k, int cus,
+                             int64_t slab_floats, int out[4]) {
+  int n = 0;
+  for (int s = 2; s <= OB_DW_SLICES_MAX; s *= 2)
+    if (ob_dw_slices_ok(k, s, cus, slab_floats)) out[n++] = s;
+  return n;
+}
diff --git a/oobleck_amd/csrc/ob_internal.h b/oobleck_amd/csrc/ob_internal.h
--- a/oobleck_amd/csrc/ob_internal.h
+++ b/oobleck_amd/csrc/ob_internal.h
@@ -243,7 +243,9 @@
   return ob_lt_shape_of(1, 0, actw, dyw, BS, lda, dyw, dyw, 1, 1.f, false,
                         false, 0);
 }
-int ob_lt_tune_shape(const ob_lt_shape& s);
+int ob_lt_tune_shape(const ob_lt_shape& s, int64_t slab_floats = 0);
+int ob_lt_dw_run(const ob_lt_shape& s, const void* act, const void* dY,
+                 float* gout, float* slab, int64_t slab_floats, void* stream);
 
 struct ob_bf16_gemm {
   const void* A = nullptr;
diff --git a/oobleck_amd/csrc/ob_layer.hip b/oobleck_amd/csrc/ob_layer.hip
--- a/oobleck_amd/csrc/ob_layer.hip
+++ b/oobleck_amd/csrc/ob_layer.hip
@@ -363,8 +363,9 @@
   if (!no_blaslt()) {
     std::vector<ob_lt_shape> shapes;
     ob_layer_lt_list(d, l->p_resid > 0.f, &shapes);
+    const int64_t slab = d->kind == OB_KIND_BLOCK ? pl.ws[WS_DW_A] : 0;
     for (const ob_lt_shape& s : shapes)
-      if (ob_lt_tune_shape(s)) return 1;
+      if (ob_lt_tune_shape(s, s.tA ? slab : 0)) return 1;
   }
   g_layers_created++;
   *out = guard.release();
@@ -692,8 +693,8 @@
                       const __bf16* dY, float* gout, void* stream) {
   const int64_t actw = s.M, dyw = s.N, BS = s.K, ldc = s.ldc;
   if (!no_blaslt()) {
-    const int r = ob_gemm_lt(s.tA, s.tB, s.M, s.N, s.K, 1.f, act, s.lda, dY,
-                             s.ldb, 1.f, gout, s.ldc, s.c_f32, stream);
+    const int r = ob_lt_dw_run(s, act, dY, gout, ws<float>(WS_DW_A),
+                               g_ws.size[WS_DW_A], stream);
     if (r >= 0) return r;
   }
   ob_bf16_gemm g;
```
